# AnishDelft/ModelCompression

Hardware: AMD Instinct MI355X
Metric: images/sec (fwd+bwd, 416x416) (higher is better)
Workload: dtype fp16

## Files before the change

### include/mcamd.h

```cpp
#ifndef MCAMD_H
#define MCAMD_H

#include <stddef.h>
#include <stdint.h>

#ifdef __cplusplus
extern "C" {
#endif

#define MCAMD_OK 0
#define MCAMD_EINVAL (-1)
#define MCAMD_ELAUNCH (-2)
#define MCAMD_EWORKSPACE (-3)

int mcamd_version(void);
void mcamd_reload_config(void);
const char* mcamd_arch(void);
const char* mcamd_last_error(void);

typedef struct mcamd_conv_geom {
    int32_t B, H, W;
    int32_t ksize;
    int32_t cin;
    int32_t cout;
// ... 102 lines not shown
                       float* wq_oihw, void* stream);
int mcamd_cast_q8_train(void* src, int64_t pixels, int32_t src_ld, int32_t src_choff, int32_t C, void* dst, int32_t dst_ld,
                        int32_t dst_choff, void* stream);

int32_t mcamd_conv_fwd_q8_sparse24_ok(const mcamd_conv_geom* g);
int mcamd_q8_sparse24_elems(const mcamd_conv_geom* g, int64_t out[3]);
int mcamd_pack_q8_sparse24(const mcamd_conv_geom* g, const float* w_oihw, const float* mask_oihw, void* wq, void* idx,
                           int32_t* wexp, void* stream);
int mcamd_conv_fwd_q8_sparse24(const mcamd_conv_geom* g, const void* x8, const void* wq, const void* idx, const int32_t* wexp,
                               const mcamd_conv_epilogue* epi, int32_t y_f8, int32_t y2_f8, void* stream);

int mcamd_conv_dgrad(const mcamd_conv_geom* g, const void* dy, int32_t dy_ld, int32_t dy_choff,
                     const void* wp_dgrad, const mcamd_conv_epilogue* epi, void* stream);

typedef struct mcamd_dgrad_sums {
    float* slab;
    int32_t rows;
    int32_t ld;
    const void* act;
    int32_t act_ld, act_choff, act_pad;
    const float* scale; const float* shift; const float* mean; const float* invstd;
    float slope;
    const float* y;
    int32_t y_ld, y_choff;
    int32_t ch_lo, C;
} mcamd_dgrad_sums;
int32_t mcamd_conv_dgrad_sums_rows(const mcamd_conv_geom* g, int32_t concurrent);
int mcamd_conv_dgrad_sums(const mcamd_conv_geom* g, const void* dy, int32_t dy_ld, int32_t dy_choff,
                          const void* wp_dgrad, const mcamd_conv_epilogue* epi, const mcamd_dgrad_sums* sums, void* stream);

size_t mcamd_conv_wgrad_workspace_bytes(const mcamd_conv_geom* g);
int mcamd_conv_wgrad(const mcamd_conv_geom* g, const void* x, const void* dy, int32_t dy_ld,
                     int32_t dy_choff, const float* mask_oihw, const mcamd_chan_map* map,
                     float grad_scale, float* dw_oihw, float* dbias, void* workspace,
                     size_t workspace_bytes, void* stream);

#define MCAMD_WGRAD_GENERIC 0
#define MCAMD_WGRAD_STEM 1
#define MCAMD_WGRAD_WIN 2
#define MCAMD_WGRAD_NINE 3
#define MCAMD_WGRAD_NINE_WIDE 4
#define MCAMD_WFIN_ROW 0
#define MCAMD_WFIN_VEC 1
#define MCAMD_WFIN_GENERIC 2
#define MCAMD_WGRAD_PLAN_INFO_N 13
int mcamd_conv_wgrad_plan_info(const mcamd_conv_geom* g, int32_t has_cmap, int32_t out[MCAMD_WGRAD_PLAN_INFO_N]);
int32_t mcamd_wgrad_generic_instances(int32_t* out, int32_t cap);

int mcamd_bn_coeffs(const float* stats, int32_t stats_rows, int32_t stats_ld, int32_t C, int64_t count,
                    const float* gamma, const float* beta, float* running_mean, float* running_var,
                    float momentum, float eps, int32_t training,
                    float* scale, float* shift, float* save_mean, float* save_invstd,
                    const int32_t* chan_perm, void* stream);

int mcamd_bn_coeffs_ex(const float* stats, int32_t stats_rows, int32_t stats_ld, int32_t C, int64_t count,
                       const float* gamma, const float* beta, float* running_mean, float* running_var,
                       float momentum, float eps, int32_t training,
                       float* scale, float* shift, float* save_mean, float* save_invstd,
                       const int32_t* chan_perm, int32_t ones_channel, void* stream);

#define MCAMD_DST_PLAIN 0
#define MCAMD_DST_POOL 1
#define MCAMD_DST_REORG 2
typedef struct mcamd_act_desc {
    int32_t B, H, W, C;
    const void* y; int32_t y_ld, y_choff;
    const float* scale; const float* shift;
    float slope;
    int32_t mode;
    void* dst; int32_t dst_ld, dst_choff;
    void* dst2; int32_t dst2_ld, dst2_choff;
    int32_t y_dtype;
    int32_t planes;
    int32_t dst_plane, dst2_plane;
    int32_t dst_pad, dst2_pad;
    const float* border;
    int32_t planes2;
    void* pool_act;
    int32_t pool_act_ld, pool_act_pad;
    void* dst_q8;
    void* dst2_q8;
} mcamd_act_desc;
int mcamd_bn_act_fwd(const mcamd_act_desc* d, void* stream);

typedef struct mcamd_act_bwd_desc {
    int32_t B, H, W, C;
    const void* y; int32_t y_ld, y_choff;
    const float* scale; const float* shift; const float* mean; const float* invstd;
    float slope;
    int32_t mode;
    const void* g; int32_t g_ld, g_choff;
    const void* g2; int32_t g2_ld, g2_choff;
    void* dy; int32_t dy_ld, dy_choff;
    float* dgamma; float* dbeta;
    float grad_scale;
    const float* dy_keep;
    const int32_t* chan_perm;
    int32_t y_dtype;
    int32_t* overflow;
    int32_t dy_pad;
    int32_t skip_dead_param_grads;
    const void* act;
    int32_t act_ld, act_choff, act_pad;
    const void* pool_out;
    int32_t pool_out_ld, pool_out_choff, pool_out_pad;
    const float* sums;
    int32_t sums_rows, sums_ld;
} mcamd_act_bwd_desc;
size_t mcamd_bn_act_bwd_workspace_bytes(const mcamd_act_bwd_desc* d);
int mcamd_bn_act_bwd(const mcamd_act_bwd_desc* d, void* workspace, size_t workspace_bytes, void* stream);

typedef struct mcamd_fold_desc {
    const float* w; const float* mask;
    const int32_t* rows; const int32_t* cols;
    const float* beta; float slope;
    int32_t n, cin_t, cin_k, cin_aug, ksize;
} mcamd_fold_desc;
int mcamd_fold_weights(const mcamd_fold_desc* d, float* waug, void* stream);
typedef struct mcamd_fold_job {
    mcamd_fold_desc d;
    float* waug;
    int64_t first_block;
} mcamd_fold_job;
int mcamd_fold_weights_many(const mcamd_fold_job* jobs_dev, int32_t njobs, int64_t total_blocks, void* stream);
int mcamd_unfold_wgrad(const mcamd_fold_desc* d, const float* dwaug, float* dw_oihw, float* prod_dbeta,
                       float* prod_dgamma, int32_t accumulate, void* stream);

typedef struct mcamd_stem_block_desc {
    int32_t B, H, W;
    const void* x;
    const void* wp;
    const float* gamma; const float* beta;
    float* running_mean; float* running_var;
    float momentum, eps;
    int32_t training;
    float* scale; float* shift; float* save_mean; float* save_invstd;
    float slope;
    void* dst; int32_t dst_ld, dst_choff;
    const void* g; int32_t g_ld, g_choff;
    const float* mask;
    float grad_scale;
    float* dw;
    float* dgamma; float* dbeta;
    int32_t cout;
    int32_t planes;
    const void* x_lo;
    const void* wp_lo;
} mcamd_stem_block_desc;
size_t mcamd_stem_block_workspace_bytes(void);
int mcamd_stem_block_fwd(const mcamd_stem_block_desc* d, void* workspace, size_t workspace_bytes, void* stream);
int mcamd_stem_block_bwd(const mcamd_stem_block_desc* d, void* workspace, size_t workspace_bytes, void* stream);
int32_t mcamd_stem_block_stats_rows(const mcamd_stem_block_desc* d);
int mcamd_stem_block_stats(const mcamd_stem_block_desc* d, float* stats, int32_t stats_rows, int32_t stats_ld, void* stream);

int mcamd_nchw_f32_to_padded_nhwc_f16(const float* src, int32_t B, int32_t C, int32_t H, int32_t W,
                                      float mul, void* dst, int32_t dst_ld, int32_t dst_choff, int32_t* overflow,
                                      void* stream);
int mcamd_nchw_f32_to_padded_nhwc_f16_pad(const float* src, int32_t B, int32_t C, int32_t H, int32_t W,
                                          float mul, void* dst, int32_t dst_ld, int32_t dst_choff, int32_t pad,
                                          int32_t* overflow, void* stream);
int mcamd_nchw_f32_to_padded_nhwc_f16_split(const float* src, int32_t B, int32_t C, int32_t H, int32_t W,
                                            void* dst, int32_t dst_ld, int32_t dst_choff, int32_t plane, void* stream);

int mcamd_nchw_f32_to_nhwc4_split(const float* src, int32_t B, int32_t H, int32_t W, void* hi, void* lo, void* stream);
int mcamd_pack_stem_split(const float* w_oihw, const float* mask_oihw, int32_t cout, void* wp_hi, void* wp_lo, void* stream);

// ... 104 lines not shown
```

### modelcompression_amd/_lib.py

```python
import ctypes as C
import os

_HERE = os.path.dirname(os.path.abspath(__file__))
LIB_PATH = os.path.join(_HERE, "libmcamd.so")


class McamdError(RuntimeError):
    pass


class ConvGeom(C.Structure):
    _fields_ = [("B", C.c_int32), ("H", C.c_int32), ("W", C.c_int32), ("ksize", C.c_int32),
                ("cin", C.c_int32), ("cout", C.c_int32), ("x_ld", C.c_int32), ("x_choff", C.c_int32),
                ("stem", C.c_int32), ("pad", C.c_int32), ("x_wrap", C.c_int32), ("x_f8", C.c_int32), ("x_f8_wexp", C.c_int32)]


class ConvEpilogue(C.Structure):
    _fields_ = [("mode", C.c_int32), ("y_ld", C.c_int32), ("y_choff", C.c_int32),
                ("y", C.c_void_p), ("bias", C.c_void_p), ("stats", C.c_void_p),
                ("stats_rows", C.c_int32), ("stats_ld", C.c_int32),
                ("scale", C.c_void_p), ("shift", C.c_void_p), ("slope", C.c_float), ("overflow", C.c_void_p),
                ("dst_mode", C.c_int32), ("y2", C.c_void_p), ("y2_ld", C.c_int32), ("y2_choff", C.c_int32),
                ("concurrent", C.c_int32)]

# ... 92 lines not shown
                ("gt_box", C.c_void_p), ("gt_cls", C.c_void_p), ("gt_difficult", C.c_void_p), ("gt_count", C.c_void_p),
                ("image_size", C.c_void_p),
                ("keys", C.c_void_p), ("flags", C.c_void_p), ("capacity", C.c_int64), ("counters", C.c_void_p)]


class FoldJob(C.Structure):
    _fields_ = [("d", FoldDesc), ("waug", C.c_void_p), ("first_block", C.c_int64)]


class AugmentDesc(C.Structure):
    _fields_ = [("src_off", C.c_int64), ("tmp_off", C.c_int64),
                ("src_w", C.c_int32), ("src_h", C.c_int32), ("crop_x", C.c_int32), ("crop_y", C.c_int32),
                ("crop_w", C.c_int32), ("crop_h", C.c_int32), ("flip", C.c_int32),
                ("hk", C.c_int32), ("vk", C.c_int32), ("hcoef_off", C.c_int32), ("vcoef_off", C.c_int32),
                ("lut_off", C.c_int32)]


class AugmentBatch(C.Structure):
    _fields_ = [("desc", C.c_void_p), ("desc_dev", C.c_void_p),
                ("src", C.c_void_p), ("src_bytes", C.c_int64),
                ("coef", C.c_void_p), ("coef_elems", C.c_int64),
                ("lut", C.c_void_p), ("lut_bytes", C.c_int64),
                ("tmp", C.c_void_p), ("tmp_bytes", C.c_int64),
                ("out", C.c_void_p), ("B", C.c_int32), ("H", C.c_int32), ("W", C.c_int32)]


EPI_RAW_F16, EPI_NCHW_F32, EPI_PAD_F16, EPI_RAW_F32 = 0, 1, 2, 3
DST_PLAIN, DST_POOL, DST_REORG = 0, 1, 2
WGRAD_GENERIC, WGRAD_STEM, WGRAD_WIN, WGRAD_NINE, WGRAD_NINE_WIDE = 0, 1, 2, 3, 4
WFIN_ROW, WFIN_VEC, WFIN_GENERIC = 0, 1, 2
WGRAD_PLAN_INFO_N = 13

_P, _I32, _I64, _F, _SZ = C.c_void_p, C.c_int32, C.c_int64, C.c_float, C.c_size_t
SIGNATURES = {
    "mcamd_version": (C.c_int, []),
    "mcamd_arch": (C.c_char_p, []),
    "mcamd_last_error": (C.c_char_p, []),
    "mcamd_reload_config": (None, []),
    "mcamd_conv_stats_rows": (_I32, [C.POINTER(ConvGeom)]),
    "mcamd_conv_stats_rows_mode": (_I32, [C.POINTER(ConvGeom), _I32]),
    "mcamd_conv_fwd_f8_ok": (_I32, [C.POINTER(ConvGeom)]),
    "mcamd_conv_tile_info": (C.c_int, [C.POINTER(ConvGeom), _I32, C.POINTER(_I32)]),
    "mcamd_conv_route_info": (C.c_int, [C.POINTER(ConvGeom), _I32, _I32, _I32, _I32, C.POINTER(_I32)]),
    "mcamd_packed_elems_fwd": (_I64, [C.POINTER(ConvGeom)]),
    "mcamd_packed_elems_dgrad": (_I64, [C.POINTER(ConvGeom)]),
    "mcamd_pack_weights": (C.c_int, [C.POINTER(ConvGeom), _P, _P, C.POINTER(ChanMap), _P, _P, _P]),
    "mcamd_pack_weights_many": (C.c_int, [_P, _I32, _I64, _P]),
    "mcamd_conv_fwd": (C.c_int, [C.POINTER(ConvGeom), _P, _P, C.POINTER(ConvEpilogue), _P]),
    "mcamd_conv_fwd_sparse24_ok": (_I32, [C.POINTER(ConvGeom)]),
    "mcamd_sparse24_elems": (C.c_int, [C.POINTER(ConvGeom), C.POINTER(_I64)]),
    "mcamd_pack_sparse24": (C.c_int, [C.POINTER(ConvGeom), _P, _P, _P, _P, _P]),
    "mcamd_conv_fwd_sparse24": (C.c_int, [C.POINTER(ConvGeom), _P, _P, _P, C.POINTER(ConvEpilogue), _P]),
    "mcamd_conv_fwd_splitk_info": (C.c_int, [C.POINTER(ConvGeom), _I32, _I32, _I32, C.POINTER(SplitkInfo)]),
    "mcamd_conv_fwd_splitk": (C.c_int, [C.POINTER(ConvGeom), _P, _P, C.POINTER(ConvEpilogue), _I32, _P, _SZ, _P]),
    "mcamd_conv_fwd_q8_ok": (_I32, [C.POINTER(ConvGeom)]),
    "mcamd_q8_elems": (C.c_int, [C.POINTER(ConvGeom), C.POINTER(_I64)]),
    "mcamd_pack_q8": (C.c_int, [C.POINTER(ConvGeom), _P, _P, _P, _P, _P]),
    "mcamd_conv_fwd_q8": (C.c_int, [C.POINTER(ConvGeom), _P, _P, _P, C.POINTER(ConvEpilogue), _I32, _I32, _P]),
    "mcamd_conv_fwd_q8_slim_ok": (_I32, [C.POINTER(ConvGeom)]),
    "mcamd_q8_slim_elems": (C.c_int, [C.POINTER(ConvGeom), C.POINTER(_I64)]),
    "mcamd_pack_q8_slim": (C.c_int, [C.POINTER(ConvGeom), _P, _P, _P, _P, _P]),
    "mcamd_conv_fwd_q8_slim": (C.c_int, [C.POINTER(ConvGeom), _P, _P, _P, C.POINTER(ConvEpilogue), _P, _I32, _I32, _I32, _P]),
    "mcamd_conv_fwd_q8_sparse24_ok": (_I32, [C.POINTER(ConvGeom)]),
    "mcamd_q8_sparse24_elems": (C.c_int, [C.POINTER(ConvGeom), C.POINTER(_I64)]),
    "mcamd_pack_q8_sparse24": (C.c_int, [C.POINTER(ConvGeom), _P, _P, _P, _P, _P, _P]),
    "mcamd_conv_fwd_q8_sparse24": (C.c_int, [C.POINTER(ConvGeom), _P, _P, _P, _P, C.POINTER(ConvEpilogue), _I32, _I32, _P]),
    "mcamd_cast_q8": (C.c_int, [_P, _I64, _I32, _I32, _I32, _P, _I32, _I32, _P]),
    "mcamd_conv_fwd_q8_stats_rows": (_I32, [C.POINTER(ConvGeom)]),
    "mcamd_fakequant_q8": (C.c_int, [C.POINTER(ConvGeom), _P, _P, _P, _P, _P]),
    "mcamd_cast_q8_train": (C.c_int, [_P, _I64, _I32, _I32, _I32, _P, _I32, _I32, _P]),
    "mcamd_conv_dgrad": (C.c_int, [C.POINTER(ConvGeom), _P, _I32, _I32, _P, C.POINTER(ConvEpilogue), _P]),
    "mcamd_conv_dgrad_sums_rows": (_I32, [C.POINTER(ConvGeom), _I32]),
    "mcamd_conv_dgrad_sums": (C.c_int, [C.POINTER(ConvGeom), _P, _I32, _I32, _P, C.POINTER(ConvEpilogue), C.POINTER(DgradSums), _P]),
    "mcamd_conv_wgrad_workspace_bytes": (_SZ, [C.POINTER(ConvGeom)]),
    "mcamd_conv_wgrad": (C.c_int, [C.POINTER(ConvGeom), _P, _P, _I32, _I32, _P, C.POINTER(ChanMap), _F, _P, _P, _P, _SZ, _P]),
    "mcamd_conv_wgrad_plan_info": (C.c_int, [C.POINTER(ConvGeom), _I32, C.POINTER(_I32)]),
    "mcamd_wgrad_generic_instances": (_I32, [C.POINTER(_I32), _I32]),
    "mcamd_bn_coeffs": (C.c_int, [_P, _I32, _I32, _I32, _I64, _P, _P, _P, _P, _F, _F, _I32, _P, _P, _P, _P, _P, _P]),
    "mcamd_bn_coeffs_ex": (C.c_int, [_P, _I32, _I32, _I32, _I64, _P, _P, _P, _P, _F, _F, _I32, _P, _P, _P, _P, _P, _I32, _P]),
    "mcamd_fold_weights": (C.c_int, [C.POINTER(FoldDesc), _P, _P]),
    "mcamd_fold_weights_many": (C.c_int, [_P, _I32, _I64, _P]),
    "mcamd_unfold_wgrad": (C.c_int, [C.POINTER(FoldDesc), _P, _P, _P, _P, _I32, _P]),
    "mcamd_bn_act_fwd": (C.c_int, [C.POINTER(ActDesc), _P]),
    "mcamd_bn_act_bwd_workspace_bytes": (_SZ, [C.POINTER(ActBwdDesc)]),
    "mcamd_bn_act_bwd": (C.c_int, [C.POINTER(ActBwdDesc), _P, _SZ, _P]),
    "mcamd_stem_block_workspace_bytes": (_SZ, []),
    "mcamd_stem_block_fwd": (C.c_int, [C.POINTER(StemBlockDesc), _P, _SZ, _P]),
    "mcamd_stem_block_bwd": (C.c_int, [C.POINTER(StemBlockDesc), _P, _SZ, _P]),
    "mcamd_stem_block_stats_rows": (_I32, [C.POINTER(StemBlockDesc)]),
    "mcamd_stem_block_stats": (C.c_int, [C.POINTER(StemBlockDesc), _P, _I32, _I32, _P]),
    "mcamd_nchw_f32_to_nhwc4_split": (C.c_int, [_P, _I32, _I32, _I32, _P, _P, _P]),
    "mcamd_pack_stem_split": (C.c_int, [_P, _P, _I32, _P, _P, _P]),
    "mcamd_nchw_f32_to_padded_nhwc_f16": (C.c_int, [_P, _I32, _I32, _I32, _I32, _F, _P, _I32, _I32, _P, _P]),
    "mcamd_nchw_f32_to_padded_nhwc_f16_pad": (C.c_int, [_P, _I32, _I32, _I32, _I32, _F, _P, _I32, _I32, _I32, _P, _P]),
    "mcamd_nchw_f32_to_padded_nhwc_f16_split": (C.c_int, [_P, _I32, _I32, _I32, _I32, _P, _I32, _I32, _I32, _P]),
    "mcamd_stem_conv_f32_stats_rows": (_I32, []),
    "mcamd_stem_conv_f32": (C.c_int, [_P, _I32, _I32, _I32, _P, _P, _I32, _P, _P, _I32, _P, _I32, _I32, _P]),
    "mcamd_region_loss_workspace_bytes": (_SZ, [_I32]),
    "mcamd_region_loss": (C.c_int, [C.POINTER(RegionDesc), _P, _P, _P, _P, _SZ, _P]),
    "mcamd_region_decode": (C.c_int, [C.POINTER(DetectDesc), _P, _P, _P]),
    "mcamd_nms": (C.c_int, [_P, _P, _I32, _I32, _F, _P, _P, _P]),
    "mcamd_detect": (C.c_int, [C.POINTER(DetectDesc), _P, _P, _P, _P, _P, _P]),
    "mcamd_voc_match": (C.c_int, [C.POINTER(VocMatchDesc), _P]),
    "mcamd_voc_ap": (C.c_int, [_P, _P, _P, _I64, _P, _I32, _P, _P, _P, _P]),
    "mcamd_augment": (C.c_int, [C.POINTER(AugmentBatch), _P]),
    "mcamd_augment_tables": (C.c_int, [_P, _P, _P, _I32, _I32, _I32, _P, _I64, _P, _I64, _P]),
    "mcamd_plan_begin": (C.c_int, [C.POINTER(_P), _I32]),
    "mcamd_plan_mark": (_I32, []),
    "mcamd_plan_end": (_P, []),
    "mcamd_plan_segments": (_I32, [_P]),
    "mcamd_plan_launches": (_I32, [_P]),
    "mcamd_plan_run": (C.c_int, [_P, _I32, _I32, C.POINTER(_P), _I32]),
    "mcamd_plan_destroy": (None, [_P]),
    "mcamd_stream_wait": (C.c_int, [_P, _P]),
    "mcamd_memset_zero": (C.c_int, [_P, _SZ, _P]),
    "mcamd_step_flags": (C.c_int, [_P, _I32, _P, _P, _P, _P, _P]),
    "mcamd_kth_magnitude_workspace_bytes": (_SZ, []),
    "mcamd_kth_magnitude": (C.c_int, [C.POINTER(_P), C.POINTER(_I64), _I32, _I64, _P, _P, _SZ, _P]),
    "mcamd_magnitude_mask": (C.c_int, [_P, _I64, _P, _P, _P]),
    "mcamd_filter_scores_workspace_bytes": (_SZ, [_I32]),
    "mcamd_filter_scores": (C.c_int, [_P, _I32, _I32, _I32, _I32, _P, _P, _SZ, _P]),
    "mcamd_filter_mean_square": (C.c_int, [_P, _I32, _I32, _I32, _I32, _P, _P, _SZ, _P]),
    "mcamd_filter_mask": (C.c_int, [_P, _I32, _I64, _P, _P]),
    "mcamd_count_zeros": (C.c_int, [_P, _I64, _P, _P]),
    "mcamd_masked_residual": (C.c_int, [_P, _P, _I64, _P, _P]),
    "mcamd_nm_mask": (C.c_int, [_P, _P, _I32, _I32, _I32, _I32, _I32, _P, _P]),
    "mcamd_nm_violations": (C.c_int, [_P, _I32, _I32, _I32, _P, _P]),
}

_lib = None


def lib():
    global _lib
    if _lib is None:
        if not os.path.exists(LIB_PATH):
            raise McamdError(
                "libmcamd.so is missing (%s). Build it with `python -m modelcompression_amd.build`; "
                "modelcompression_amd has no CPU/PyTorch fallback for its compute path." % LIB_PATH)
        import torch
        h = C.CDLL(LIB_PATH)
        for name, (res, args) in SIGNATURES.items():
            fn = getattr(h, name)
            fn.restype = res
            fn.argtypes = args
        _lib = h
    return _lib


def reload_config():
    lib().mcamd_reload_config()


def check(rc, what=""):
    if rc != 0:
        msg = lib().mcamd_last_error().decode()
        raise McamdError("%s failed (%d): %s" % (what or "mcamd call", rc, msg))


def ptr(t):
    return None if t is None else C.c_void_p(t.data_ptr())


def stream_ptr():
    import torch
    return C.c_void_p(torch.cuda.current_stream().cuda_stream)
# ... 1 lines not shown
```

### modelcompression_amd/build.py

```python
import os
import subprocess
import sys
from concurrent.futures import ThreadPoolExecutor

HERE = os.path.dirname(os.path.abspath(__file__))
CSRC = os.path.join(HERE, "csrc")
OUT = os.path.join(HERE, "libmcamd.so")
HIPCC = os.environ.get("HIPCC", "/opt/rocm/bin/hipcc")
ARCH = "gfx950"
COMMON = ["--offload-arch=" + ARCH, "-O3", "-fPIC", "-std=c++17", "-Wall", "-Wno-unused-variable",
          "-fhip-fp32-correctly-rounded-divide-sqrt"]
SOURCES = {
    "api.hip": [],
    "conv_igemm.hip": [],
    "conv_igemm_pp.hip": [],
    "conv_sparse.hip": [],
    "conv_splitk.hip": [],
    "conv_q8.hip": [],
    "conv_q8_sparse.hip": [],
    "conv_stem.hip": [],
    "conv_stem_block.hip": [],
    "conv_stem_f32.hip": [],
    "conv_small.hip": [],
    "conv_win.hip": [],
    "conv_wres.hip": [],
    "conv_wgrad.hip": [],
    "conv_wgrad_stem.hip": [],
    "bn_act.hip": [],
    "fold.hip": [],
    "plan.hip": [],
    "region_loss.hip": [],
    "prune.hip": ["-ffp-contract=off"],
    "augment.hip": ["-ffp-contract=off"],
    "detect.hip": ["-ffp-contract=off"],
    "voc_eval.hip": ["-ffp-contract=off"],
}


def _stale(target, deps):
    if not os.path.exists(target):
        return True
    t = os.path.getmtime(target)
    return any(os.path.getmtime(d) > t for d in deps)


def build(force=False, verbose=False):
    headers = [os.path.join(CSRC, f) for f in os.listdir(CSRC) if f.endswith(".h")]
    headers.append(os.path.join(os.path.dirname(HERE), "include", "mcamd.h"))
    objdir = os.path.join(CSRC, "build")
    os.makedirs(objdir, exist_ok=True)
    jobs = []
    for src, extra in SOURCES.items():
        s = os.path.join(CSRC, src)
        o = os.path.join(objdir, src.replace(".hip", ".o"))
        if force or _stale(o, [s] + headers):
            jobs.append([HIPCC] + COMMON + extra + ["-c", s, "-o", o])

    def run(cmd):
        if verbose:
            print(" ".join(cmd))
        r = subprocess.run(cmd, capture_output=True, text=True)
        if r.returncode != 0:
            raise RuntimeError("hipcc failed:\n%s\n%s" % (" ".join(cmd), r.stderr))
        return r.stderr

    with ThreadPoolExecutor(max_workers=4) as ex:
        for err in ex.map(run, jobs):
            if verbose and err.strip():
                print(err)
    objs = [os.path.join(objdir, s.replace(".hip", ".o")) for s in SOURCES]
    if force or jobs or _stale(OUT, objs):
        run([HIPCC, "--offload-arch=" + ARCH, "-shared", "-fPIC", "-o", OUT] + objs)
    return OUT


if __name__ == "__main__":
    print(build(force="--force" in sys.argv, verbose=True))
```

### modelcompression_amd/csrc/api.hip

```cpp
#include <stdarg.h>
#include <stdlib.h>
#include <string.h>

#include "kernels.h"

static thread_local char g_err[512] = "";

void mcamd_set_error(const char* fmt, ...) {
    va_list ap;
    va_start(ap, fmt);
    vsnprintf(g_err, sizeof(g_err), fmt, ap);
    va_end(ap);
}

int g_mcamd_env_generation = 0;
int McamdEnvSlot::get(const char* name, int dflt) {
    const int g = __atomic_load_n(&g_mcamd_env_generation, __ATOMIC_ACQUIRE);
    if (gen != g) {
        const char* s = getenv(name);
        has = s && *s ? 1 : 0;
        val = has ? atoi(s) : 0;
        __atomic_store_n(&gen, g, __ATOMIC_RELEASE);
    }
    return has ? val : dflt;
}
extern "C" void mcamd_reload_config(void) { __atomic_add_fetch(&g_mcamd_env_generation, 1, __ATOMIC_ACQ_REL); }

extern "C" int mcamd_version(void) { return 101; }
extern "C" const char* mcamd_arch(void) { return "gfx950"; }
extern "C" const char* mcamd_last_error(void) { return g_err; }

static int cin_tap_of(const mcamd_conv_geom* g) { return g->stem ? 32 : round_up_int(g->cin, 32); }
static int ntaps_of(const mcamd_conv_geom* g) { return g->stem ? 3 : g->ksize * g->ksize; }
static int cout_p_of(const mcamd_conv_geom* g) { return round_up_int(g->cout, 32); }
static int pw_of(const mcamd_conv_geom* g) { return g->pad ? 1 : 2; }
static long long padded_pixels(const mcamd_conv_geom* g) {
    const int pw = pw_of(g);
    return (long long)g->B * (g->H + pw) * (g->W + pw) + (pw == 1 ? g->W + 2 : 0);
}

static int check_geom(const mcamd_conv_geom* g, const char* what) {
    MCAMD_REQUIRE(g, "%s: null geometry", what);
    MCAMD_REQUIRE(g->B > 0 && g->H > 0 && g->W > 0 && g->cin > 0 && g->cout > 0, "%s: non-positive dimension", what);
    MCAMD_REQUIRE(g->ksize == 1 || g->ksize == 3, "%s: ksize %d unsupported (1 or 3)", what, g->ksize);
    MCAMD_REQUIRE((long long)g->B * g->H * g->W < (1ll << 31), "%s: more than 2^31 output pixels", what);
    MCAMD_REQUIRE(g->pad == 0 || (g->pad == 1 && !g->stem), "%s: pad must be 0 or 1 (and 0 for the stem layer)", what);
    if (g->stem) {
        MCAMD_REQUIRE(g->cin == 3 && g->ksize == 3 && g->x_ld == 4 && g->x_choff == 0,
                      "%s: stem form needs cin=3, ksize=3, x_ld=4, x_choff=0", what);
    } else {
        MCAMD_REQUIRE(g->x_ld % 8 == 0 && g->x_choff % 8 == 0, "%s: x_ld / x_choff must be multiples of 8", what);
        const int span = g->x_wrap > 0 ? g->x_wrap : cin_tap_of(g);
        MCAMD_REQUIRE(g->x_choff + span <= g->x_ld, "%s: x channel slice [%d, %d) exceeds x_ld %d", what,
                      g->x_choff, g->x_choff + span, g->x_ld);
    }
    if (g->x_f8 != 0) {
        MCAMD_REQUIRE(!g->stem && g->x_wrap == 0 && g->x_f8 > 0 && g->x_f8 % 64 == 0 && g->cin == 2 * g->x_f8 && g->x_choff == 0,
                      "%s: x_f8 %d needs cin = 2 P with P %% 64 == 0, no x_wrap, x_choff 0 (cin %d, x_choff %d)", what, g->x_f8, g->cin,
                      g->x_choff);
        MCAMD_REQUIRE(g->x_f8_wexp >= -24 && g->x_f8_wexp <= 40, "%s: x_f8_wexp %d outside [-24, 40]", what, g->x_f8_wexp);
    }
    if (g->x_wrap != 0) {
        const int ct = cin_tap_of(g), kb = ct % 64 == 0 ? 64 : 32;
        MCAMD_REQUIRE(!g->stem && g->x_wrap > 0 && g->x_wrap % 64 == 0 && g->x_wrap % kb == 0 && g->cin == g->x_wrap / 2 * 3 && ct == g->cin,
                      "%s: x_wrap %d needs cin = 3 P, x_wrap = 2 P, P %% 32 == 0 (cin %d)", what, g->x_wrap, g->cin);
    }
    return MCAMD_OK;
}

static void fill_taps(int ksize, int stem, int row_stride, int ld, int* taps) {
    if (stem) {
        for (int ty = 0; ty < 3; ++ty) taps[ty] = ty * row_stride;
    } else if (ksize == 3) {
        for (int ty = 0; ty < 3; ++ty)
            for (int tx = 0; tx < 3; ++tx) taps[ty * 3 + tx] = ty * row_stride + tx * ld;
    } else {
        taps[0] = row_stride + ld;
    }
}

extern "C" int64_t mcamd_packed_elems_fwd(const mcamd_conv_geom* g) {
    if (!g) return 0;
    return (int64_t)round_up_int(g->cout, 256) * ntaps_of(g) * cin_tap_of(g);
}
extern "C" int64_t mcamd_packed_elems_dgrad(const mcamd_conv_geom* g) {
// ... 374 lines not shown
    if (mcamd_win3x3_ok(mode, stats, M, n, ct, ktot, g->H, g->W))
        return {ROUTE_WIN3X3, 32, round_up_int(n, 16), 64, 0};
    if (fwd && g->x_f8 > 0 && mode == MCAMD_EPI_RAW_F32) ct = ct / 2 * 3, ktot = ktot / 2 * 3;
    return mcamd_igemm_route(M, n, ct, ktot, mode == MCAMD_EPI_RAW_F16, dir == DIR_DGRAD_CONCURRENT);
}

static int launch_route(IgemmArgs& a, const ConvRoute& r, const mcamd_conv_geom* g, hipStream_t st) {
    switch (r.kernel) {
    case ROUTE_STEM: {
        StemArgs q;
        q.x = a.x, q.w = a.w, q.y = (half_t*)a.y, q.stats = a.stats;
        q.y_ld = a.y_ld, q.y_choff = a.y_choff, q.stats_ld = a.stats_ld;
        q.H = g->H, q.W = g->W, q.HW = a.HW, q.M = a.M;
        return mcamd_stem_launch(q, g->cout, r.rows, st);
    }
    case ROUTE_WRES: return mcamd_wres_launch(a, g->B, r.rows, st);
    case ROUTE_SMALL3X3_SPLIT: return mcamd_small3x3_split_launch(a, r.rows, st);
    case ROUTE_SMALL3X3: return mcamd_small3x3_launch(a, r.rows, st);
    case ROUTE_WIN3X3: return mcamd_win3x3_launch(a, st);
    default: return mcamd_igemm_launch(a, r, st);
    }
}

extern "C" int32_t mcamd_conv_stats_rows_mode(const mcamd_conv_geom* g, int32_t mode) {
    if (!g) return 0;
    return conv_route(g, DIR_FWD, mode == MCAMD_EPI_RAW_F32 ? MCAMD_EPI_RAW_F32 : MCAMD_EPI_RAW_F16, MCAMD_DST_PLAIN, true).rows;
}

extern "C" int32_t mcamd_conv_stats_rows(const mcamd_conv_geom* g) { return mcamd_conv_stats_rows_mode(g, MCAMD_EPI_RAW_F16); }

extern "C" int32_t mcamd_conv_fwd_f8_ok(const mcamd_conv_geom* g) {
    if (!g || g->x_f8 <= 0 || g->x_f8 % 64 != 0 || g->cin != 2 * g->x_f8 || g->stem || g->x_wrap != 0 || g->x_choff != 0) return 0;
    return conv_route(g, DIR_FWD, MCAMD_EPI_RAW_F32, MCAMD_DST_PLAIN, true).kernel == ROUTE_PP ? 1 : 0;
}

extern "C" int mcamd_conv_tile_info(const mcamd_conv_geom* g, int32_t dgrad, int32_t out[4]) {
    if (check_geom(g, "conv_tile_info")) return MCAMD_EINVAL;
    MCAMD_REQUIRE(out, "conv_tile_info: null output");
    const bool f32 = !dgrad && (g->x_wrap > 0 || g->x_f8 > 0);
    const ConvRoute r = conv_route(g, dgrad, f32 ? MCAMD_EPI_RAW_F32 : MCAMD_EPI_RAW_F16, MCAMD_DST_PLAIN, !dgrad);
    out[0] = r.bm, out[1] = r.bn, out[2] = r.bk, out[3] = r.kernel;
    return MCAMD_OK;
}

extern "C" int mcamd_conv_route_info(const mcamd_conv_geom* g, int32_t dir, int32_t mode, int32_t dst_mode, int32_t stats,
                                     int32_t out[5]) {
    if (check_geom(g, "conv_route_info")) return MCAMD_EINVAL;
    MCAMD_REQUIRE(out, "conv_route_info: null output");
    MCAMD_REQUIRE(dir == DIR_FWD || dir == DIR_DGRAD || dir == DIR_DGRAD_CONCURRENT, "conv_route_info: bad direction %d", dir);
    MCAMD_REQUIRE(mode >= MCAMD_EPI_RAW_F16 && mode <= MCAMD_EPI_RAW_F32, "conv_route_info: bad epilogue mode %d", mode);
    MCAMD_REQUIRE(dst_mode == MCAMD_DST_PLAIN || dst_mode == MCAMD_DST_POOL || dst_mode == MCAMD_DST_REORG,
                  "conv_route_info: bad dst_mode %d", dst_mode);
    const ConvRoute r = conv_route(g, dir, mode, dst_mode, stats != 0);
    out[0] = r.bm, out[1] = r.bn, out[2] = r.bk, out[3] = r.kernel, out[4] = r.rows;
    return MCAMD_OK;
}

extern "C" int mcamd_conv_fwd(const mcamd_conv_geom* g, const void* x, const void* wp_fwd, const mcamd_conv_epilogue* epi,
                              void* stream) {
    if (mcamd_recording()) {
        MCAMD_REQUIRE(g && epi, "conv_fwd: null geometry / epilogue");
        const mcamd_conv_geom g_ = *g;
        const mcamd_conv_epilogue e_ = *epi;
        return mcamd_rec_push(stream, [=](void* s) { return mcamd_conv_fwd(&g_, x, wp_fwd, &e_, s); });
    }
    if (check_geom(g, "conv_fwd")) return MCAMD_EINVAL;
    MCAMD_REQUIRE(x && wp_fwd && epi, "conv_fwd: null input / epilogue");
    IgemmArgs a;
    fill_operand(a, g, x, wp_fwd, g->x_ld, g->x_choff, g->cout, cin_tap_of(g), g->stem);
    MCAMD_REQUIRE(g->x_wrap == 0 || epi->mode == MCAMD_EPI_RAW_F32 || epi->mode == MCAMD_EPI_NCHW_F32,
                  "conv_fwd: x_wrap goes with the fp32 epilogues (modes 3 and 1)");
    if (g->x_wrap > 0) a.wrap = g->x_wrap;
    if (g->x_f8 > 0) a.f8_from = (g->x_f8 / a.kb) * a.ntaps * (a.kb / 32);
    a.f8_sb = (127 - (MCAMD_F8_SXL + g->x_f8_wexp)) * 0x01010101;
    const ConvRoute r = conv_route(g, DIR_FWD, epi->mode, epi->dst_mode, epi->stats != nullptr);
    if (g->x_f8 > 0) {
        MCAMD_REQUIRE(epi->mode == MCAMD_EPI_RAW_F32, "conv_fwd: x_f8 goes with the fp32 epilogue (mode 3)");
        MCAMD_REQUIRE(r.kernel == ROUTE_PP, "conv_fwd: no fp8-correction kernel for this shape (mcamd_conv_fwd_f8_ok)");
    }
    if (fill_epilogue(a, epi, g->cout, "conv_fwd", r.rows)) return MCAMD_EINVAL;
    return launch_route(a, r, g, (hipStream_t)stream);
}

extern "C" int32_t mcamd_conv_fwd_sparse24_ok(const mcamd_conv_geom* g) {
    if (!g || g->stem || g->x_wrap != 0 || g->x_f8 != 0 || (g->ksize != 1 && g->ksize != 3)) return 0;
    if (g->B <= 0 || g->H <= 0 || g->W <= 0 || g->cin <= 0 || g->cout <= 0) return 0;
    if (g->cin % 4 != 0 || g->cout % 8 != 0 || (long long)g->B * g->H * g->W >= (1ll << 31)) return 0;
    if (g->pad != 0 && g->pad != 1) return 0;
    if (g->x_ld % 8 != 0 || g->x_choff % 8 != 0 || g->x_choff + cin_tap_of(g) > g->x_ld) return 0;
    return 1;
}

extern "C" int mcamd_sparse24_elems(const mcamd_conv_geom* g, int64_t out[2]) {
    MCAMD_REQUIRE(g && out, "sparse24_elems: null argument");
    MCAMD_REQUIRE(mcamd_conv_fwd_sparse24_ok(g), "sparse24_elems: geometry has no 2:4 form (mcamd_conv_fwd_sparse24_ok)");
    const long long npad = round_up_int(g->cout, 256), ktot = (long long)ntaps_of(g) * cin_tap_of(g);
    out[0] = npad * ktot / 2;
    out[1] = npad * ktot / 16;
    return MCAMD_OK;
}

extern "C" int mcamd_pack_sparse24(const mcamd_conv_geom* g, const float* w_oihw, const float* mask_oihw, void* wsp, void* idx,
                                   void* stream) {
    if (mcamd_recording()) {
        MCAMD_REQUIRE(g, "pack_sparse24: null geometry");
        const mcamd_conv_geom g_ = *g;
        return mcamd_rec_push(stream, [=](void* s) { return mcamd_pack_sparse24(&g_, w_oihw, mask_oihw, wsp, idx, s); });
    }
    MCAMD_REQUIRE(g && mcamd_conv_fwd_sparse24_ok(g), "pack_sparse24: geometry has no 2:4 form (mcamd_conv_fwd_sparse24_ok)");
    MCAMD_REQUIRE(w_oihw && wsp && idx, "pack_sparse24: null pointer");
    const int ct = cin_tap_of(g);
    return mcamd_pack_sparse24_launch(w_oihw, mask_oihw, wsp, idx, g->cout, g->cin, ntaps_of(g), ct, kblock_of(ct),
                                      (hipStream_t)stream);
}

extern "C" int mcamd_conv_fwd_sparse24(const mcamd_conv_geom* g, const void* x, const void* wsp, const void* idx,
                                       const mcamd_conv_epilogue* epi, void* stream) {
    if (mcamd_recording()) {
        MCAMD_REQUIRE(g && epi, "conv_fwd_sparse24: null geometry / epilogue");
        const mcamd_conv_geom g_ = *g;
        const mcamd_conv_epilogue e_ = *epi;
        return mcamd_rec_push(stream, [=](void* s) { return mcamd_conv_fwd_sparse24(&g_, x, wsp, idx, &e_, s); });
    }
    if (check_geom(g, "conv_fwd_sparse24")) return MCAMD_EINVAL;
    MCAMD_REQUIRE(mcamd_conv_fwd_sparse24_ok(g), "conv_fwd_sparse24: geometry has no 2:4 form (mcamd_conv_fwd_sparse24_ok)");
    MCAMD_REQUIRE(x && wsp && idx, "conv_fwd_sparse24: null input");
    MCAMD_REQUIRE(epi && epi->mode == MCAMD_EPI_PAD_F16, "conv_fwd_sparse24: epilogue mode 2 (MCAMD_EPI_PAD_F16) only");
    IgemmArgs a;
    fill_operand(a, g, x, wsp, g->x_ld, g->x_choff, g->cout, cin_tap_of(g), 0);
    if (fill_epilogue(a, epi, g->cout, "conv_fwd_sparse24", 0)) return MCAMD_EINVAL;
    return mcamd_sparse24_launch(a, idx, (hipStream_t)stream);
}

static int splitk_plan_for(const mcamd_conv_geom* g, int mode, int dst_mode, int slices, const char* what, SplitkPlan* p) {
    MCAMD_REQUIRE(g, "%s: null geometry", what);
    MCAMD_REQUIRE(g->stem == 0, "%s: stem %d: the first layer has no split-K form", what, g->stem);
    MCAMD_REQUIRE(g->pad == 0, "%s: pad %d: the shared-halo form is not accepted (pad must be 0)", what, g->pad);
    MCAMD_REQUIRE(g->x_wrap == 0, "%s: x_wrap %d: split operands have no split-K form", what, g->x_wrap);
    MCAMD_REQUIRE(g->x_f8 == 0, "%s: x_f8 %d: the fp8 correction form has no split-K form", what, g->x_f8);
    if (check_geom(g, what)) return MCAMD_EINVAL;
    MCAMD_REQUIRE(mode == MCAMD_EPI_PAD_F16 || mode == MCAMD_EPI_RAW_F16,
                  "%s: epilogue mode %d: modes 2 (MCAMD_EPI_PAD_F16) and 0 (MCAMD_EPI_RAW_F16) only", what, mode);
    MCAMD_REQUIRE(dst_mode == MCAMD_DST_PLAIN || (mode == MCAMD_EPI_PAD_F16 && (dst_mode == MCAMD_DST_POOL || dst_mode == MCAMD_DST_REORG)),
                  "%s: bad dst_mode %d for epilogue mode %d", what, dst_mode, mode);
    MCAMD_REQUIRE(slices >= 0, "%s: slices %d is negative", what, slices);
    const int ct = cin_tap_of(g);
    *p = mcamd_splitk_plan((long long)g->B * g->H * g->W, g->cout, ct, ntaps_of(g) * ct, slices);
    MCAMD_REQUIRE(p->slices >= 1 && p->slices <= p->chunks, "%s: slices %d outside [1, chunks = %d]", what, p->slices, p->chunks);
    return MCAMD_OK;
}

extern "C" int mcamd_conv_fwd_splitk_info(const mcamd_conv_geom* g, int32_t mode, int32_t dst_mode, int32_t slices,
                                          mcamd_splitk_info* out) {
    MCAMD_REQUIRE(out, "conv_fwd_splitk_info: null output");
    SplitkPlan p;
    if (splitk_plan_for(g, mode, dst_mode, slices, "conv_fwd_splitk_info", &p)) return MCAMD_EINVAL;
    out->slices = p.slices;
    out->bm = p.bm, out->bn = p.bn, out->bk = p.bk;
    out->chunks = p.chunks;
    out->tiles = p.tiles;
    out->workspace_bytes = (int64_t)p.slices * p.slab_elems * (int64_t)sizeof(float);
    return MCAMD_OK;
}

extern "C" int mcamd_conv_fwd_splitk(const mcamd_conv_geom* g, const void* x, const void* wp_fwd, const mcamd_conv_epilogue* epi,
                                     int32_t slices, void* workspace, size_t workspace_bytes, void* stream) {
// ... 379 lines not shown
```

### modelcompression_amd/csrc/bn_act.hip

```cpp
#include "common.h"
#include "conv_epi.h"

constexpr int RED_CPB = 8, RED_RG = 128;

__device__ __forceinline__ double shfl_xor_f64(double v, int m) {
    int lo = __double2loint(v), hi = __double2hiint(v);
    lo = __shfl_xor(lo, m);
    hi = __shfl_xor(hi, m);
    return __hiloint2double(hi, lo);
}

__device__ __forceinline__ void block_reduce2(double& a, double& b, double (*red)[16][RED_CPB]) {
    const int lane = threadIdx.x & 63, wave = threadIdx.x >> 6, cx = threadIdx.x & (RED_CPB - 1);
#pragma unroll
    for (int m = RED_CPB; m < 64; m <<= 1) {
        a += shfl_xor_f64(a, m);
        b += shfl_xor_f64(b, m);
    }
    if (lane < RED_CPB) {
        red[0][wave][cx] = a;
        red[1][wave][cx] = b;
    }
    __syncthreads();
    if (threadIdx.x < RED_CPB) {
        a = b = 0.0;
        for (int w = 0; w < 16; ++w) {
            a += red[0][w][cx];
            b += red[1][w][cx];
        }
    }
}

__global__ __launch_bounds__(1024) void bn_coeffs_kernel(const float* stats, int rows, int ld, int C, double count,
                                                         const float* gamma, const float* beta, float* rmean,
                                                         float* rvar, float momentum, float eps, int training,
                                                         float* scale, float* shift, float* save_mean,
                                                         float* save_invstd, const int* perm, int ones_channel) {
    __shared__ double red[2][16][RED_CPB];
    const int cx = threadIdx.x & (RED_CPB - 1), ry = threadIdx.x / RED_CPB;
    const int c = blockIdx.x * RED_CPB + cx;
    double s1 = 0.0, s2 = 0.0;
    if (training && c < C) {
        for (int p = ry; p < rows; p += RED_RG) {
            s1 += (double)stats[((long long)p * 2 + 0) * ld + c];
            s2 += (double)stats[((long long)p * 2 + 1) * ld + c];
        }
    }
    block_reduce2(s1, s2, red);
    if (ry != 0 || c >= C) return;
    const int pc = perm ? perm[c] : c;
    double mean, var;
    if (training) {
        mean = s1 / count;
        var = s2 / count - mean * mean;
        if (var < 0.0) var = 0.0;
        double unbiased = count > 1.0 ? var * count / (count - 1.0) : var;
        rmean[pc] = (float)((1.0 - momentum) * (double)rmean[pc] + (double)momentum * mean);
        rvar[pc] = (float)((1.0 - momentum) * (double)rvar[pc] + (double)momentum * unbiased);
    } else {
        mean = rmean[pc];
        var = rvar[pc];
    }
    double invstd = 1.0 / sqrt(var + (double)eps);
    float sc = (float)((double)gamma[pc] * invstd);
    scale[c] = sc;
    shift[c] = (float)((double)beta[pc] - mean * (double)sc);
    if (c == ones_channel) scale[c] = 0.f, shift[c] = 1.f;
    if (save_mean) save_mean[c] = (float)mean;
    if (save_invstd) save_invstd[c] = (float)invstd;
}

struct ActArgs {
    const void* y;
    const float* scale;
    const float* shift;
    half_t* dst;
    half_t* dst2;
    int B, H, W, C;
    int y_ld, y_choff, dst_ld, dst_choff, dst2_ld, dst2_choff;
    float slope;
    long long items;
    const float* border;
    int dst_plane, dst2_plane;
    int dst_pw, dst2_pw;
    int dst2_pl;
    half_t* pool_act;
    int pool_act_ld, pool_act_pw;
    char* dst_q8;
    char* dst2_q8;
};

__device__ __forceinline__ void load8(const half_t* p, float* v) {
    h8_t h = *(const h8_t*)p;
#pragma unroll
    for (int i = 0; i < 8; ++i) v[i] = (float)h[i];
}
__device__ __forceinline__ half_t sat_half(float v) {
    return (half_t)fminf(fmaxf(v, -65504.f), 65504.f);
}
__device__ __forceinline__ void store8(half_t* p, const float* v) {
    h8_t h;
#pragma unroll
    for (int i = 0; i < 8; ++i) h[i] = sat_half(v[i]);
    *(h8_t*)p = h;
}
__device__ __forceinline__ void loadf8(const float* p, float* v) {
    f32x4_t a = *(const f32x4_t*)p, b = *(const f32x4_t*)(p + 4);
#pragma unroll
    for (int i = 0; i < 4; ++i) {
        v[i] = a[i];
        v[4 + i] = b[i];
    }
}
template <bool Y32>
__device__ __forceinline__ void load_y(const void* y, long long idx, float* v) {
    if (Y32) loadf8((const float*)y + idx, v);
    else load8((const half_t*)y + idx, v);
}
template <int PL>
__device__ __forceinline__ void store_act(half_t* p, int plane, const float* v, int ci = 0) {
    h8_t hi;
#pragma unroll
    for (int i = 0; i < 8; ++i) hi[i] = sat_half(v[i]);
    *(h8_t*)p = hi;
    if (PL == 4) {
        float ql[8], q8[8];
#pragma unroll
        for (int i = 0; i < 8; ++i) {
            ql[i] = fminf(fmaxf((v[i] - (float)hi[i]) * (float)(1 << MCAMD_F8_SXL), -448.f), 448.f);
            q8[i] = fminf(fmaxf(v[i] * (float)(1 << MCAMD_F8_SX8), -448.f), 448.f);
        }
        int wl[2], w8[2];
#pragma unroll
        for (int i = 0; i < 2; ++i) {
            wl[i] = __builtin_amdgcn_cvt_pk_fp8_f32(ql[4 * i], ql[4 * i + 1], 0, false);
            wl[i] = __builtin_amdgcn_cvt_pk_fp8_f32(ql[4 * i + 2], ql[4 * i + 3], wl[i], true);
            w8[i] = __builtin_amdgcn_cvt_pk_fp8_f32(q8[4 * i], q8[4 * i + 1], 0, false);
            w8[i] = __builtin_amdgcn_cvt_pk_fp8_f32(q8[4 * i + 2], q8[4 * i + 3], w8[i], true);
        }
        char* b = (char*)(p - ci + plane) + ci;
        typedef int i32x2_t __attribute__((ext_vector_type(2)));
        *(i32x2_t*)b = i32x2_t{wl[0], wl[1]};
        *(i32x2_t*)(b + plane) = i32x2_t{w8[0], w8[1]};
    } else if (PL >= 2) {
        h8_t lo;
#pragma unroll
        for (int i = 0; i < 8; ++i) lo[i] = (half_t)(v[i] - (float)hi[i]);
        *(h8_t*)(p + plane) = lo;
        if (PL == 3) *(h8_t*)(p + 2 * plane) = hi;
    }
}
__device__ __forceinline__ void store_act_q8(half_t* p, char* q, long long off, const float* v) {
    if (!q) {
        store_act<1>(p + off, 0, v);
        return;
    }
    i32x2_t o;
    o[0] = e4m3_bytes4(v), o[1] = e4m3_bytes4(v + 4);
    *(i32x2_t*)(q + off) = o;
    h8_t h = q8_to_f16(o[0], o[1]);
#pragma unroll
    for (int i = 0; i < 8; ++i) h[i] = h[i] * (half_t)0.5f;
    *(h8_t*)(p + off) = h;
}
__device__ __forceinline__ unsigned short half_prev_bits(unsigned short b) {
    if (b == 0x0000 || b == 0x8000) return 0x8001;
    return (b & 0x8000) ? (unsigned short)(b + 1) : (unsigned short)(b - 1);
}
template <int PL>
__device__ __forceinline__ void store_act2(int pl2, half_t* p, int plane, const float* v, int ci) {
    if (PL < 2 || pl2 == PL) store_act<PL>(p, plane, v, ci);
    else if (pl2 == 4) store_act<4>(p, plane, v, ci);
    else if (pl2 == 3) store_act<3>(p, plane, v, ci);
    else if (pl2 == 2) store_act<2>(p, plane, v, ci);
    else store_act<1>(p, plane, v, ci);
}

__device__ __forceinline__ int border_class(int h, int w, int H, int W) {
    return (h == 0 ? 1 : 0) | (h == H - 1 ? 2 : 0) | (w == 0 ? 4 : 0) | (w == W - 1 ? 8 : 0);
}

template <int MODE, bool FIXED, bool Y32, int PL, bool Q8 = false>
__global__ __launch_bounds__(256) void bn_act_fwd_kernel(ActArgs a) {
    const int CH = a.C >> 3;
    int c8 = (threadIdx.x % CH) * 8;
    float sc[8], sh[8];
    if (FIXED) {
        loadf8(a.scale + c8, sc);
        loadf8(a.shift + c8, sh);
    }
    const int Ho = a.H >> 1, Wo = a.W >> 1;
    for (long long item = (long long)blockIdx.x * 256 + threadIdx.x; item < a.items; item += (long long)gridDim.x * 256) {
        long long pix = item / CH;
        if (!FIXED) {
            c8 = (int)(item - pix * CH) * 8;
            loadf8(a.scale + c8, sc);
            loadf8(a.shift + c8, sh);
        }
        if (MODE == MCAMD_DST_PLAIN) {
            int b = (int)(pix / (a.H * a.W));
            int rem = (int)(pix - (long long)b * a.H * a.W);
            int h = rem / a.W, w = rem - h * a.W;
            float v[8];
            load_y<Y32>(a.y, pix * a.y_ld + a.y_choff + c8, v);
            if (a.border) {
                float bb[8];
                loadf8(a.border + border_class(h, w, a.H, a.W) * a.C + c8, bb);
#pragma unroll
                for (int i = 0; i < 8; ++i) v[i] += bb[i];
            }
#pragma unroll
            for (int i = 0; i < 8; ++i) {
                float z = v[i] * sc[i] + sh[i];
                v[i] = z > 0.f ? z : z * a.slope;
            }
            if (Q8) store_act_q8(a.dst, a.dst_q8, pad_off(b, h, w, a.H, a.W, a.dst_ld, a.dst_pw) + a.dst_choff + c8, v);
            else store_act<PL>(a.dst + pad_off(b, h, w, a.H, a.W, a.dst_ld, a.dst_pw) + a.dst_choff + c8, a.dst_plane, v, a.dst_choff + c8);
        } else {
            int b = (int)(pix / (Ho * Wo));
            int rem = (int)(pix - (long long)b * Ho * Wo);
            int ho = rem / Wo, wo = rem - ho * Wo;
            float act[4][8];
#pragma unroll
            for (int k = 0; k < 4; ++k) {
                int h = 2 * ho + (k >> 1), w = 2 * wo + (k & 1);
                long long sp = ((long long)b * a.H + h) * a.W + w;
                load_y<Y32>(a.y, sp * a.y_ld + a.y_choff + c8, act[k]);
                if (a.border) {
                    float bb[8];
                    loadf8(a.border + border_class(h, w, a.H, a.W) * a.C + c8, bb);
#pragma unroll
                    for (int i = 0; i < 8; ++i) act[k][i] += bb[i];
                }
#pragma unroll
                for (int i = 0; i < 8; ++i) {
                    float z = act[k][i] * sc[i] + sh[i];
                    act[k][i] = z > 0.f ? z : z * a.slope;
                }
                if (Q8) {
                    if (a.dst2) store_act_q8(a.dst2, a.dst2_q8, pad_off(b, h, w, a.H, a.W, a.dst2_ld, a.dst2_pw) + a.dst2_choff + c8, act[k]);
                } else if (a.dst2) store_act2<PL>(a.dst2_pl, a.dst2 + pad_off(b, h, w, a.H, a.W, a.dst2_ld, a.dst2_pw) + a.dst2_choff + c8, a.dst2_plane, act[k], a.dst2_choff + c8);
            }
            long long dp = pad_off(b, ho, wo, Ho, Wo, a.dst_ld, a.dst_pw) + a.dst_choff;
            if (MODE == MCAMD_DST_POOL) {
                float m[8];
#pragma unroll
                for (int i = 0; i < 8; ++i) m[i] = fmaxf(fmaxf(act[0][i], act[1][i]), fmaxf(act[2][i], act[3][i]));
                if (Q8) store_act_q8(a.dst, a.dst_q8, dp + c8, m);
                else store_act<PL>(a.dst + dp + c8, a.dst_plane, m, a.dst_choff + c8);
                if (!Q8 && a.pool_act) {
                    typedef unsigned short us8_t __attribute__((ext_vector_type(8)));
                    us8_t hb[4];
#pragma unroll
                    for (int i = 0; i < 8; ++i) {
                        int arg = 0;
                        float best = act[0][i];
#pragma unroll
                        for (int k = 1; k < 4; ++k) {
                            const bool gt = act[k][i] > best;
                            best = gt ? act[k][i] : best, arg = gt ? k : arg;
                        }
                        const unsigned short top = __builtin_bit_cast(unsigned short, sat_half(best));
                        const unsigned short below = half_prev_bits(top);
#pragma unroll
                        for (int k = 0; k < 4; ++k) {
                            const unsigned short hk = __builtin_bit_cast(unsigned short, sat_half(act[k][i]));
                            hb[k][i] = (k != arg && hk == top) ? below : hk;
                        }
                    }
                    half_t* q0 = a.pool_act + pad_off(b, 2 * ho, 2 * wo, a.H, a.W, a.pool_act_ld, a.pool_act_pw) + c8;
                    const long long qrow = (long long)(a.W + a.pool_act_pw) * a.pool_act_ld;
                    *(us8_t*)q0 = hb[0];
                    *(us8_t*)(q0 + a.pool_act_ld) = hb[1];
                    *(us8_t*)(q0 + qrow) = hb[2];
                    *(us8_t*)(q0 + qrow + a.pool_act_ld) = hb[3];
                }
            } else {
#pragma unroll
                for (int k = 0; k < 4; ++k) {
                    if (Q8) store_act_q8(a.dst, a.dst_q8, dp + k * a.C + c8, act[k]);
                    else store_act<PL>(a.dst + dp + k * a.C + c8, a.dst_plane, act[k], a.dst_choff + k * a.C + c8);
                }
            }
        }
    }
}

struct ActBwdArgs {
    const void* y;
    const float* scale;
    const float* shift;
    const float* mean;
    const float* invstd;
    const half_t* g;
    const half_t* g2;
    half_t* dy;
    float* slab;
    const float* coef;
    const float* dy_keep;
    int* overflow;
    int B, H, W, C;
    int y_ld, y_choff, g_ld, g_choff, g2_ld, g2_choff, dy_ld, dy_choff;
    float slope;
    long long items;
    int dy_pw;
    const half_t* act;
    int act_ld, act_choff, act_pw;
    const half_t* pool_out;
    int pool_out_ld, pool_out_choff, pool_out_pw;
};

__device__ __forceinline__ void block_partials_to_slab(const float (&sb)[8], const float (&sg)[8], int CH, float* slab, int C) {
    constexpr int PITCH = 264;
    __shared__ float red[16 * PITCH];
#pragma unroll
    for (int i = 0; i < 8; ++i) {
        red[i * PITCH + threadIdx.x] = sb[i];
        red[(8 + i) * PITCH + threadIdx.x] = sg[i];
    }
    __syncthreads();
    const int reps = 256 / CH;
// ... 1102 lines not shown
```

### modelcompression_amd/csrc/conv_epi.h

```cpp
#pragma once
#include "kernels.h"

__device__ __forceinline__ void split_image(int p, int HW, int& b, int& hw) {
    b = p / HW;
    hw = p - b * HW;
}
__device__ __forceinline__ void split_pixel(int p, int HW, int W, int& b, int& h, int& w) {
    int r;
    split_image(p, HW, b, r);
    h = r / W;
    w = r - h * W;
}

__device__ __forceinline__ void tile_pixel(const IgemmArgs& __restrict__ a, bool pooled, int m, int& b, int& h, int& w) {
    if (pooled) {
        const int Wo = a.W >> 1, q = m & 3;
        int ho, wo;
        split_pixel(m >> 2, (a.H >> 1) * Wo, Wo, b, ho, wo);
        h = 2 * ho + (q >> 1);
        w = 2 * wo + (q & 1);
    } else {
        split_pixel(m, a.HW, a.W, b, h, w);
    }
}
// ... 47 lines not shown
template <int ROWS, int COLS, int PITCH, int NT>
__device__ __forceinline__ void store_pad_tile(const IgemmArgs& __restrict__ a, const char* bt, const half_t* ht, bool y_f8, bool y2_f8,
                                               int mt, int nt, int tid) {
    constexpr int CH = COLS / 8;
    if (a.dst_mode == MCAMD_DST_PLAIN) {
        for (int slot = tid; slot < ROWS * CH; slot += NT) {
            const int row = slot / CH, ch = slot - row * CH;
            const int m = mt * ROWS + row;
            const int n0 = nt * COLS + ch * 8;
            if (m < a.M && n0 < a.N) {
                int b, h, w;
                split_pixel(m, a.HW, a.W, b, h, w);
                put8(a.y, y_f8, pad_off(b, h, w, a.H, a.W, a.y_ld) + a.y_choff + n0, bt, ht, row * PITCH + ch * 8);
            }
        }
        return;
    }
    const int Wo = a.W >> 1, Ho = a.H >> 1, HWo = Ho * Wo;
    if (a.dst_mode == MCAMD_DST_POOL) {
        const bool has2 = a.y2 != nullptr;
        for (int slot = tid; slot < (ROWS / 4) * CH; slot += NT) {
            const int pr = slot / CH, ch = slot - pr * CH;
            const int idx = mt * (ROWS / 4) + pr;
            const int n0 = nt * COLS + ch * 8;
            if (4 * idx < a.M && n0 < a.N) {
                int b, ho, wo;
                split_pixel(idx, HWo, Wo, b, ho, wo);
                const long long off = pad_off(b, ho, wo, Ho, Wo, a.y_ld) + a.y_choff + n0;
                if (y_f8) {
                    unsigned k0 = 0, k1 = 0;
#pragma unroll
                    for (int q = 0; q < 4; ++q) {
                        const i32x2_t v = *(const i32x2_t*)(bt + (4 * pr + q) * PITCH + ch * 8);
                        k0 = e4m3_max4(k0, e4m3_key((unsigned)v[0]));
                        k1 = e4m3_max4(k1, e4m3_key((unsigned)v[1]));
                    }
                    i32x2_t mx;
                    mx[0] = (int)e4m3_unkey(k0), mx[1] = (int)e4m3_unkey(k1);
                    *(i32x2_t*)((char*)a.y + off) = mx;
                } else {
                    h8_t v[4];
#pragma unroll
                    for (int q = 0; q < 4; ++q) v[q] = *(const h8_t*)(ht + (4 * pr + q) * PITCH + ch * 8);
                    h8_t mx;
#pragma unroll
                    for (int e = 0; e < 8; ++e) {
                        const half_t m01 = v[0][e] > v[1][e] ? v[0][e] : v[1][e], m23 = v[2][e] > v[3][e] ? v[2][e] : v[3][e];
                        mx[e] = m01 > m23 ? m01 : m23;
                    }
                    *(h8_t*)((half_t*)a.y + off) = mx;
                }
                if (has2) {
#pragma unroll
                    for (int q = 0; q < 4; ++q)
                        put8(a.y2, y2_f8, pad_off(b, 2 * ho + (q >> 1), 2 * wo + (q & 1), a.H, a.W, a.y2_ld) + a.y2_choff + n0,
                             bt, ht, (4 * pr + q) * PITCH + ch * 8);
                }
            }
        }
    } else {
        for (int slot = tid; slot < ROWS * CH; slot += NT) {
            const int row = slot / CH, ch = slot - row * CH;
            const int m = mt * ROWS + row;
            const int n0 = nt * COLS + ch * 8;
            if (m < a.M && n0 < a.N) {
                int b, ho, wo;
                split_pixel(m >> 2, HWo, Wo, b, ho, wo);
                put8(a.y, y_f8, pad_off(b, ho, wo, Ho, Wo, a.y_ld) + a.y_choff + (m & 3) * a.N + n0, bt, ht, row * PITCH + ch * 8);
            }
        }
    }
}

template <int ROWS, int COLS, int NT>
__device__ __forceinline__ void store_raw_tile(const IgemmArgs& __restrict__ a, const half_t* ct, int mt, int nt, int tid) {
    constexpr int CH = COLS / 8;
    half_t* y = (half_t*)a.y;
    for (int slot = tid; slot < ROWS * CH; slot += NT) {
        const int row = slot / CH, ch = slot - row * CH;
        const int m = mt * ROWS + row;
        const int n0 = nt * COLS + ch * 8;
        if (m < a.M && n0 < a.N) *(h8_t*)(y + (long long)m * a.y_ld + a.y_choff + n0) = *(const h8_t*)(ct + row * COLS + ch * 8);
    }
}

template <class T>
__device__ __forceinline__ const T* pin_here(const T* p) {
    asm volatile("" : "+s"(p));
    return p;
}
__host__ __device__ constexpr int sums_vals(int cols, int nt) { return (2 * cols + nt - 1) / nt; }
__host__ __device__ constexpr size_t sums_lds_bytes(int nt) { return (size_t)16 * (nt + 8) * sizeof(float); }

__host__ __device__ constexpr int sums_slots(int rows, int cols, int nt) { return rows * (cols / 8) / nt; }
__host__ __device__ constexpr int sums_early(int rows, int cols, int nt) {
    return rows * cols >= 256 * 256 && sums_slots(rows, cols, nt) > 8 ? 8 : sums_slots(rows, cols, nt);
}

template <int ROWS, int COLS, int NT>
__device__ __forceinline__ void sums_prefetch(const IgemmArgs& __restrict__ a, int mt, int nt, int tid,
                                              h8_t (&aq)[sums_early(ROWS, COLS, NT)]) {
    constexpr int CH = COLS / 8, RSTEP = NT / CH, NSLOT = sums_early(ROWS, COLS, NT);
    static_assert(NT % CH == 0 && (ROWS * CH) % NT == 0, "a thread keeps its 8 channels for all its slots");
    const int ch = tid % CH, row0 = tid / CH;
    const int n0 = nt * COLS + ch * 8;
    const int c = n0 - a.bsum.ch_lo;
    const bool live = n0 < a.N && c >= 0 && c < a.bsum.C;
    const half_t* act = pin_here(a.bsum.act) + a.bsum.act_choff + c;
    int m = mt * ROWS + row0;
    int b, h, w;
    split_pixel(m, a.HW, a.W, b, h, w);
    const int sb_ = RSTEP / a.HW, srem = RSTEP - sb_ * a.HW;
    const int sh_ = srem / a.W, sw_ = srem - sh_ * a.W;
#pragma unroll
    for (int k = 0; k < NSLOT; ++k) {
#pragma unroll
        for (int i = 0; i < 8; ++i) aq[k][i] = (half_t)0.f;
        if (live && m < a.M) aq[k] = *(const h8_t*)(act + pad_off(b, h, w, a.H, a.W, a.bsum.act_ld, a.bsum.act_pw));
        m += RSTEP;
        w += sw_;
        if (w >= a.W) w -= a.W, ++h;
        h += sh_;
        if (h >= a.H) h -= a.H, ++b;
        b += sb_;
    }
}

template <int ROWS, int COLS, int NT>
__device__ __forceinline__ void store_raw_tile_sums(const IgemmArgs& __restrict__ a, char* smem, int mt, int nt, int tid,
                                                    const h8_t (&aq)[sums_early(ROWS, COLS, NT)],
                                                    float (&tot)[sums_vals(COLS, NT)]) {
    constexpr int CH = COLS / 8, RSTEP = NT / CH, NSLOT = sums_slots(ROWS, COLS, NT), PITCH = NT + 8;
    constexpr int EARLY = sums_early(ROWS, COLS, NT);
    const half_t* ct = (const half_t*)smem;
    half_t* y = (half_t*)a.y;
    const int ch = tid % CH, row0 = tid / CH;
    const int n0 = nt * COLS + ch * 8;
    const int c = n0 - a.bsum.ch_lo;
    const bool col_ok = n0 < a.N;
    const bool live = col_ok && c >= 0 && c < a.bsum.C;
    float sb[8], sg[8], off[8], mul[8];
    bool usey[8];
    bool need_y = false;
#pragma unroll
    for (int i = 0; i < 8; ++i) sb[i] = sg[i] = 0.f, off[i] = 0.f, mul[i] = 0.f, usey[i] = false;
    if (live) {
        const float *scp = pin_here(a.bsum.scale) + c, *shp = pin_here(a.bsum.shift) + c;
        const float *mup = pin_here(a.bsum.mean) + c, *isp = pin_here(a.bsum.invstd) + c;
        float sc[8], sh[8], mu[8], is[8];
#pragma unroll
        for (int i = 0; i < 8; ++i) sc[i] = scp[i], sh[i] = shp[i], mu[i] = mup[i], is[i] = isp[i];
        need_y = act_xhat_source(sc, sh, mu, is, a.bsum.y != nullptr, off, mul, usey);
    }
    const float slope = a.bsum.slope, inv_slope = 1.0f / slope;
#pragma unroll
    for (int k = 0; k < NSLOT; ++k) {
        const int row = row0 + k * RSTEP, m = mt * ROWS + row;
        if (!col_ok || m >= a.M) continue;
        const h8_t gq = *(const h8_t*)(ct + row * COLS + ch * 8);
        *(h8_t*)(y + (long long)m * a.y_ld + a.y_choff + n0) = gq;
        if (!live) continue;
        h8_t av8;
        if (k < EARLY) {
            av8 = aq[k];
        } else {
            int b, h, w;
// ... 136 lines not shown
```

### modelcompression_amd/csrc/conv_igemm.hip

```cpp
#include "kernels.h"
#include "conv_epi.h"
#include <stdlib.h>


template <int BM, int BN, int WM, int WN, int BK, int NSTAGE, int EPI>
__global__ __launch_bounds__((BM / WM) * (BN / WN) * 64,
                              (BN >= 128 ? (NSTAGE * BK <= 96 ? 3 : 2) : (BN >= 64 ? 3 : 4)))
void igemm_kernel(IgemmArgs a) {
    constexpr int WAVES_N = BN / WN;
    constexpr int NT = (BM / WM) * (BN / WN) * 64;
    constexpr int CPR = BK / 8;
    constexpr int A_SLOTS = BM * CPR, B_SLOTS = BN * CPR;
    constexpr int A_IT = (A_SLOTS + NT - 1) / NT, B_IT = (B_SLOTS + NT - 1) / NT;
    constexpr int TM = WM / 32, TN = WN / 32;
    constexpr int STAGE_BYTES = (A_SLOTS + B_SLOTS) * 16;
    constexpr int DMIN = A_SLOTS / NT + B_SLOTS / NT;
    static_assert(A_SLOTS % 64 == 0 && B_SLOTS % 64 == 0, "whole waves per DMA instruction");
    static_assert(NSTAGE >= 2 && NSTAGE <= 4 && DMIN * (NSTAGE - 2) < 64, "vmcnt immediate range");

    extern __shared__ __attribute__((aligned(16))) char smem[];

    const int tid = threadIdx.x;
    const int lane = tid & 63;
    const int wave = __builtin_amdgcn_readfirstlane(tid >> 6);
// ... 67 lines not shown
                int wslot = it * NT + wave * 64;
                if (wslot < B_SLOTS) glds16(a.w + bbase[it] + (long long)q * BK, sb + wslot * 16);
            }
        };

        __syncthreads();
#pragma unroll
        for (int p = 0; p < NSTAGE - 1; ++p)
            if (p < nchunks) stage(p, p);
        int sidx = 0;
        for (int q = 0; q < nchunks; ++q) {
            int issued = q + NSTAGE - 1;
            if (issued > nchunks) issued = nchunks;
            const int inflight = issued - q - 1;
            if (NSTAGE == 2 || inflight == 0) wait_vmcnt<0>();
            else if (inflight == 1) wait_vmcnt<DMIN>();
            else wait_vmcnt<(NSTAGE > 3 ? 2 * DMIN : DMIN)>();
            __builtin_amdgcn_s_barrier();
            if (q + NSTAGE - 1 < nchunks) {
                int ns = sidx + NSTAGE - 1;
                if (ns >= NSTAGE) ns -= NSTAGE;
                stage(q + NSTAGE - 1, ns);
            }
            const char* sa = smem + sidx * STAGE_BYTES;
            const char* sb = sa + A_SLOTS * 16;
            sidx = sidx + 1 == NSTAGE ? 0 : sidx + 1;
            constexpr int KS = BK / 16;
            constexpr int NSET = (TM * TN <= 4) ? 2 : 1;
            h8_t af[NSET][TM], bf[NSET][TN];
            auto load_frags = [&](int s, int set) {
                const int chunk = 2 * s + (lane >> 5);
#pragma unroll
                for (int i = 0; i < TM; ++i) {
                    int row = wm * WM + i * 32 + (lane & 31);
                    af[set][i] = *(const h8_t*)(sa + (row * CPR + (chunk ^ swz<CPR>(row))) * 16);
                }
#pragma unroll
                for (int j = 0; j < TN; ++j) {
                    int row = wn * WN + j * 32 + (lane & 31);
                    bf[set][j] = *(const h8_t*)(sb + (row * CPR + (chunk ^ swz<CPR>(row))) * 16);
                }
            };
            if (NSET == 2) load_frags(0, 0);
#pragma unroll
            for (int s = 0; s < KS; ++s) {
                if (NSET == 2) {
                    if (s + 1 < KS) load_frags(s + 1, (s + 1) & 1);
                    __builtin_amdgcn_sched_barrier(0);
                } else {
                    load_frags(s, 0);
                }
                constexpr int M1 = NSET - 1;
#pragma unroll
                for (int i = 0; i < TM; ++i)
#pragma unroll
                    for (int j = 0; j < TN; ++j)
                        acc[i][j] = __builtin_amdgcn_mfma_f32_32x32x16_f16(af[s & M1][i], bf[s & M1][j], acc[i][j], 0, 0, 0);
                if (NSET == 2) __builtin_amdgcn_sched_barrier(0);
            }
        }

        if constexpr (EPI == MCAMD_EPI_NCHW_F32) {
            float* y = (float*)a.y;
#pragma unroll
            for (int i = 0; i < TM; ++i)
#pragma unroll
                for (int r = 0; r < 16; ++r) {
                    int m = mt * BM + wm * WM + i * 32 + mfma32_row(r, lane);
                    if (m < a.M) {
                        int b, hw;
                        split_image(m, a.HW, b, hw);
#pragma unroll
                        for (int j = 0; j < TN; ++j) {
                            int n = nt * BN + wn * WN + j * 32 + (lane & 31);
                            if (n < a.N) {
                                float v = acc[i][j][r];
                                if (a.bias) v += a.bias[n];
                                y[((long long)b * a.N + n) * a.HW + hw] = v;
                            }
                        }
                    }
                }
        } else if constexpr (EPI == MCAMD_EPI_RAW_F32) {
            float* y = (float*)a.y;
            const int mlim = a.M - mt * BM;
#pragma unroll
            for (int j = 0; j < TN; ++j) {
                const int n = nt * BN + wn * WN + j * 32 + (lane & 31);
#pragma unroll
                for (int i = 0; i < TM; ++i)
#pragma unroll
                    for (int r = 0; r < 16; ++r) {
                        const int row = wm * WM + i * 32 + mfma32_row(r, lane);
                        const float v = acc[i][j][r];
                        if (row < mlim) {
                            if (n < a.N) y[(long long)(mt * BM + row) * a.y_ld + a.y_choff + n] = v;
                            s1[j] += v;
                            s2[j] += v * v;
                        }
                    }
            }
        } else {
            h8_t aq[SUMS ? sums_early(BM, BN, NT) : 1];
            if constexpr (SUMS) sums_prefetch<BM, BN, NT>(a, mt, nt, tid, aq);
            __syncthreads();
            half_t* ct = (half_t*)smem;
            const int mlim = a.M - mt * BM;
#pragma unroll
            for (int j = 0; j < TN; ++j) {
                const int col = wn * WN + j * 32 + (lane & 31);
                float sc = 1.f, sh = 0.f;
                if constexpr (EPI == MCAMD_EPI_PAD_F16) {
                    int n = nt * BN + col;
                    if (n < a.N) {
                        if (a.scale) sc = a.scale[n];
                        if (a.shift) sh = a.shift[n];
                    }
                }
#pragma unroll
                for (int i = 0; i < TM; ++i)
#pragma unroll
                    for (int r = 0; r < 16; ++r) {
                        const int row = wm * WM + i * 32 + mfma32_row(r, lane);
                        float v = acc[i][j][r];
                        if constexpr (EPI == MCAMD_EPI_PAD_F16) {
                            v = v * sc + sh;
                            v = v > 0.f ? v : v * a.slope;
                        }
                        half_t hv = (half_t)fminf(fmaxf(v, -65504.f), 65504.f);
                        sat |= fabsf(v) > 65504.f;
                        ct[row * BN + col] = hv;
                        if (EPI == MCAMD_EPI_RAW_F16 && a.stats) {
                            float fv = (row < mlim) ? (float)hv : 0.f;
                            s1[j] += fv;
                            s2[j] += fv * fv;
                        }
                    }
            }
            __syncthreads();
            if constexpr (EPI == MCAMD_EPI_PAD_F16) store_pad_tile<BM, BN, BN, NT>(a, nullptr, ct, false, false, mt, nt, tid);
            else if constexpr (SUMS) store_raw_tile_sums<BM, BN, NT>(a, smem, mt, nt, tid, aq, tot);
            else store_raw_tile<BM, BN, NT>(a, ct, mt, nt, tid);
        }
    }

    if (sat && a.overflow) atomicOr(a.overflow, 1);
    if constexpr (SUMS) store_tile_sums_slab<BN, NT>(a, pslot, nt, tid, tot);
    if ((EPI == MCAMD_EPI_RAW_F16 || EPI == MCAMD_EPI_RAW_F32) && a.stats) {
#pragma unroll
        for (int j = 0; j < TN; ++j) {
            s1[j] += __shfl_xor(s1[j], 32);
            s2[j] += __shfl_xor(s2[j], 32);
        }
        __syncthreads();
        float* red = (float*)smem;
        if (lane < 32) {
#pragma unroll
            for (int j = 0; j < TN; ++j) {
                red[(wm * 2 + 0) * BN + wn * WN + j * 32 + lane] = s1[j];
                red[(wm * 2 + 1) * BN + wn * WN + j * 32 + lane] = s2[j];
            }
        }
        __syncthreads();
        for (int t = tid; t < 2 * BN; t += NT) {
            int which = t / BN, col = t - which * BN;
            float v = 0.f;
#pragma unroll
            for (int k = 0; k < BM / WM; ++k) v += red[(k * 2 + which) * BN + col];
            a.stats[((long long)pslot * 2 + which) * a.stats_ld + nt * BN + col] = v;
        }
    }
}

struct TileCfg {
    int bm, bn, bk;
    int kind;
};

static TileCfg pick_tile(long long M, int n, int cin_tap, int ktot, bool raw_epilogue = true, bool concurrent = false) {
    TileCfg t;
    t.kind = 0;
    if (raw_epilogue && mcamd_small3x3_ok(M, n, cin_tap, ktot)) {
        t.bm = 32, t.bn = round_up_int(n, 32), t.bk = cin_tap, t.kind = 4;
        return t;
    }
    {
        const int pp = MCAMD_ENV_INT("MCAMD_PP", 1);
        if (pp && ktot >= 256 && n >= 128 && M >= 256) {
            bool use = pp == 2;
            int bm = 256, bn = 256;
            if (pp == 1 && ktot >= 1152) {
                double best_cost = -1.0, best_span = 0.0;
                const int bms[2] = {256, 192}, bns[2] = {256, 128};
                for (int cn = 0; cn < 2; ++cn) {
                    if (n < bns[cn]) continue;
                    for (int c = 0; c < 2; ++c) {
                        const long long tiles = ((M + bms[c] - 1) / bms[c]) * ((n + bns[cn] - 1) / bns[cn]);
                        const long long rounds = (tiles + 255) / 256;
                        const double fill = (double)tiles / (double)(rounds * 256);
                        const double rate = bns[cn] == 256 ? 1.0 : 0.8;
                        if (fill < 0.8 && !(concurrent && rounds == 1 && fill >= 0.4)) continue;
                        const double span = (double)rounds * bms[c] * bns[cn] / rate;
                        const double cost = concurrent ? (double)tiles * bms[c] * bns[cn] / rate : span;
                        const bool better = best_cost < 0 || (concurrent ? (cost < 0.97 * best_cost || (cost < 1.03 * best_cost && span < best_span))
                                                                         : cost < best_cost);
                        if (better) best_cost = cost, best_span = span, bm = bms[c], bn = bns[cn];
                    }
                }
                use = best_cost >= 0;
            }
            if (pp >= 2) {
                if (MCAMD_ENV_INT("MCAMD_PP_BM", 256) == 192) bm = 192;
                if (MCAMD_ENV_INT("MCAMD_PP_BN", 256) == 128) bn = 128;
            }
            if (use) {
                t.bm = bm, t.bn = bn, t.bk = 32, t.kind = 2;
                return t;
            }
        }
    }
    int best = 128, waste = round_up_int(n, 128);
    for (int bn = 64; bn >= 32; bn /= 2)
        if (round_up_int(n, bn) < waste) {
            waste = round_up_int(n, bn);
            best = bn;
        }
    t.bm = 128;
    t.bn = best;
    if (t.bn == 128 && (n % 64 == 0 || round_up_int(n, 64) == round_up_int(n, 128))) {
        const long long t128 = ((M + 127) / 128) * ((n + 127) / 128);
        if (t128 < 256 && 2 * t128 <= 512) t.bn = 64;
    }
    int want_bk = MCAMD_ENV_INT("MCAMD_BK", 64);
    t.bk = (want_bk == 64 && cin_tap % 64 == 0) ? 64 : 32;
    if (t.bm == 128 && t.bn == 128 && t.bk == 64 && ktot >= 2048) {
        const long long nt = (n + 127) / 128;
        const long long t128 = ((M + 127) / 128) * nt, t192 = ((M + 191) / 192) * nt;
        const long long cost128 = ((t128 + 511) / 512) * 128, cost192 = ((t192 + 511) / 512) * 192;
        if (cost192 <= cost128) t.bm = 192;
    }
    return t;
}

static int igemm_mtiles(long long M, int bm) { return (int)((M + bm - 1) / bm); }

ConvRoute mcamd_igemm_route(long long M, int n, int cin_tap, int ktot, bool raw_epilogue, bool concurrent) {
    const TileCfg t = pick_tile(M, n, cin_tap, ktot, raw_epilogue, concurrent);
    if (t.kind == ROUTE_SMALL3X3) return {t.kind, t.bm, t.bn, t.bk, mcamd_small3x3_rows(M)};
    int ntiles = (n + t.bn - 1) / t.bn;
    int mtiles = igemm_mtiles(M, t.bm);
    int target = t.kind == ROUTE_PP ? 256 : 2048;
    int p = target / ntiles;
    if (p < 1) p = 1;
    if (p > mtiles) p = mtiles;
// ... 61 lines not shown
```

### modelcompression_amd/csrc/kernels.h

```cpp
#pragma once
#include "common.h"

struct DgradSums {
    float* slab;
    const half_t* act;
    const float* scale;
    const float* shift;
    const float* mean;
    const float* invstd;
    const float* y;
    int act_ld, act_choff, act_pw;
    int y_ld, y_choff;
    int ch_lo, C;
    int ld;
    float slope;
};
#define MCAMD_EPI_RAW_F16_SUMS 4

struct IgemmArgs {
    const half_t* x;
    const half_t* w;
    void* y;
    const float* bias;
    float* stats;
// ... 49 lines not shown
    int dy_zero_off;
    int H, W, HW, M;
    int rows_pad;
    int ktot, cin_tap, ntaps;
    int tap_off[9];
    int n_ctiles;
    int n_otiles, n_tapgroups, nsplit;
    int pix_per_split;
};

struct WgradPlan {
    int tmo, tnc, taps, kp, rows_pad, n_otiles, n_ctiles, n_tapgroups, nsplit, pix_per_split;
    int nine;
    int stemw;
    int ns;
    size_t bytes;
};

struct WgradFinish {
    int kernel;
    int sg;
};

enum { ROUTE_IGEMM = 0, ROUTE_STEM = 1, ROUTE_PP = 2, ROUTE_SMALL3X3 = 4, ROUTE_WIN3X3 = 5, ROUTE_WRES = 6, ROUTE_SMALL3X3_SPLIT = 7 };
struct ConvRoute {
    int kernel;
    int bm, bn, bk;
    int rows;
};

ConvRoute mcamd_igemm_route(long long M, int n, int cin_tap, int ktot, bool raw_epilogue, bool concurrent);
int mcamd_igemm_pp_launch(const IgemmArgs& a, int bm, int bn, int rows, int ntiles, hipStream_t st);
int mcamd_igemm_launch(IgemmArgs& a, const ConvRoute& r, hipStream_t st);
bool mcamd_igemm_sums_ok(const ConvRoute& r);
struct SplitkPlan {
    int bm, bn, bk, chunks, mtiles, ntiles, tiles, slices;
    long long slab_elems;
};
SplitkPlan mcamd_splitk_plan(long long M, int n, int cin_tap, int ktot, int forced);
int mcamd_splitk_launch(const IgemmArgs& a, const SplitkPlan& p, float* ws, hipStream_t st);
int mcamd_sparse24_launch(IgemmArgs& a, const void* idx, hipStream_t st);
int mcamd_pack_sparse24_launch(const float* w, const float* mask, void* vals, void* idx, int cout, int cin, int ntaps,
                               int cin_tap, int kb, hipStream_t st);
int mcamd_conv_q8_launch(IgemmArgs& a, const void* wexp, int y_f8, int y2_f8, hipStream_t st, const float* border = nullptr,
                         int border_ld = 0);
int mcamd_pack_q8_launch(const float* w, const float* mask, void* wq, void* wexp, int cout, int cin, int ntaps, hipStream_t st);
int mcamd_pack_q8_slim_launch(const float* w, const float* mask, void* wq, void* wexp, int cout, int cin, int ntaps, hipStream_t st);
#define MCAMD_Q8_TILE_M 128
int mcamd_cast_q8_launch(const void* src, long long pixels, int src_ld, int src_choff, int C, void* dst, int dst_ld,
                         int dst_choff, int back, hipStream_t st);
int mcamd_fakequant_q8_launch(const float* w, const float* mask, const void* wexp, float* out, int cout, int cin, int ntaps,
                              hipStream_t st);
int mcamd_conv_q8_sparse_launch(IgemmArgs& a, const void* idx, const void* wexp, int y_f8, int y2_f8, hipStream_t st);
int mcamd_pack_q8_sparse24_launch(const float* w, const float* mask, void* wq, void* idx, void* wexp, int cout, int cin,
                                  int ntaps, hipStream_t st);

WgradPlan mcamd_wgrad_plan(long long M, int cout, int cin_tap, int ntaps);
int mcamd_wgrad_launch(WgradArgs& a, const WgradPlan& p, hipStream_t st);
bool mcamd_wgrad_stem_ok(int stem, int cout, int W, long long M);
WgradPlan mcamd_wgrad_stem_plan(long long M);
int mcamd_wgrad_stem_launch(WgradArgs& a, const WgradPlan& p, hipStream_t st);
bool mcamd_wgrad_win_ok(int ksize, int stem, int cout, int cin_tap, int W, long long M);
WgradPlan mcamd_wgrad_win_plan(long long M, int cout);
int mcamd_wgrad_win_launch(WgradArgs& a, const WgradPlan& p, hipStream_t st);
bool mcamd_wgrad_use9(int ksize, int stem, int cout, int cin_tap, int W);
WgradPlan mcamd_wgrad_plan9(long long P, int cout, int cin_tap, int W, int pitch, int B);
int mcamd_wgrad9_launch(const WgradArgs& w, const WgradPlan& p, int pitch, long long P, hipStream_t st);
WgradFinish mcamd_wgrad_finish_pick(int nsplit, int stem, int Cin, int ksize, bool has_cmap);
int mcamd_wgrad_instances(int (*out)[4], int cap);
int mcamd_wgrad_finish_launch(const float* slab, const WgradPlan& p, int ktot, int cin_tap, int stem, int Cout, int Cin,
                              int ksize, const float* mask, float inv_scale, float* dw, const int* rmap, const int* cmap,
                              hipStream_t st);
int mcamd_colsum_launch(const half_t* dy, long long rows, int ld, int choff, int C, float inv_scale, float* out,
                        hipStream_t st, void* scratch, size_t scratch_bytes);

bool mcamd_win3x3_ok(int mode, bool stats, long long M, int n, int cin_tap, int ktot, int H, int W);
int mcamd_win3x3_launch(const IgemmArgs& a, hipStream_t st);
bool mcamd_small3x3_ok(long long M, int n, int cin_tap, int ktot);
int mcamd_small3x3_rows(long long M);
int mcamd_small3x3_launch(const IgemmArgs& a, int rows, hipStream_t st);
bool mcamd_small3x3_split_ok(long long M, int n, int cin_tap, int ktot, int wrap, int mode);
int mcamd_small3x3_split_launch(const IgemmArgs& a, int rows, hipStream_t st);

bool mcamd_wres_ok(int ksize, int stem, int n, int cin_tap, int ktot, int B, int H, int W, int mode);
int mcamd_wres_rows(int n, int B, int H, int W);
int mcamd_wres_launch(IgemmArgs& a, int B, int rows, hipStream_t st);

bool mcamd_stem_direct_ok(int stem, int cout, int mode);
int mcamd_stem_rows(long long M);
int mcamd_stem_launch(const StemArgs& a, int cout, int rows, hipStream_t st);
```

### modelcompression_amd/engine.py

```python
import contextlib
import math
import os
import time

import torch

from . import ops
from . import _lib as L
from ._lib import McamdError


class _T:
    __slots__ = ("buf", "ld", "choff", "C", "H", "W", "ps", "ps0")

    def __init__(self, buf, ld, choff, C, H, W, ps=0):
        self.buf, self.ld, self.choff, self.C, self.H, self.W, self.ps = buf, ld, choff, C, H, W, ps
        self.ps0 = ps


class _Layer:
    pass


def _resolve_routes(blocks):
# ... 15 lines not shown
PLAIN_BLOCK_ERR = 2.9e-4
MIXED_BUDGET = 5.5e-4
MIXED_BUDGET_TRAIN = 7.0e-4
TRAIN_GAIN = 1.1


def _probe_side_stream(device, tries=8):
    lock = None
    try:
        import fcntl
        import tempfile
        lock = open(os.path.join(tempfile.gettempdir(), "mcamd_side_probe.lock"), "w")
        fcntl.flock(lock, fcntl.LOCK_EX)
    except Exception:
        lock = None
    try:
        main = torch.cuda.current_stream(device)
        big = torch.empty(64 << 20, dtype=torch.float32, device=device)
        tiny = torch.zeros(64, dtype=torch.float32, device=device)
        first = None
        for _ in range(tries):
            cand = torch.cuda.Stream(device)
            first = first or cand
            torch.cuda.synchronize(device)
            busy, done = torch.cuda.Event(enable_timing=True), torch.cuda.Event(enable_timing=True)
            for _ in range(80):
                big.fill_(1.0)
            busy.record(main)
            with torch.cuda.stream(cand):
                tiny.add_(1.0)
                done.record(cand)
            torch.cuda.synchronize(device)
            concurrent = done.elapsed_time(busy) > 0.0
            if concurrent:
                return cand, True
        return first, False
    finally:
        if lock is not None:
            try:
                import fcntl
                fcntl.flock(lock, fcntl.LOCK_UN)
                lock.close()
            except Exception:
                pass


class Engine:
    def __init__(self, model, B, H, W, device, grad_scale=256.0, precision="fp16", for_training=False, train_layout=False):
        if precision not in ("fp16", "fp16x3", "mixed", "fp8", "fp8-2:4", "fp8-qat"):
            raise McamdError("precision must be 'fp16', 'fp16x3', 'mixed', 'fp8', 'fp8-2:4' or 'fp8-qat' (got %r)" % (precision,))
        self.model, self.B, self.device = model, B, device
        self.precision = precision
        self.for_training = bool(for_training)
        self.train_layout = bool(train_layout)
        self.precise = precision not in ("fp16", "fp8", "fp8-2:4", "fp8-qat")
        self.q8 = precision in ("fp8", "fp8-2:4", "fp8-qat")
        self.qat = precision == "fp8-qat"
        self.fp8_layers = []
        self.q8_sparse = precision == "fp8-2:4"
        self.fp8_sparse_layers = []
        self.qbufs = {}
        self._qld = {}
        self._q8_keys = None
        self.grad_scale = float(grad_scale)
        self.serial = 0
        self._packed_sig = None
        self.events = None
        self.overlap_wgrad = os.environ.get("MCAMD_OVERLAP_WGRAD", "1") == "1"
        self.wgrad_chunk = 1
        self.use_plan = os.environ.get("MCAMD_PLAN", "1") == "1"
        self._fwd_plans, self._bwd_plan, self._plan_epoch = {}, None, 0
        self._logits = self._gout = self._flat = None
        self._pack_on_side = False
        self.sparse_layers = []
        self._sparse_mode, self._sparse_keys = None, None
        self.splitk_layers = []
        self._splitk_on, self._splitk_keys, self._splitk_ws = False, None, None
        self.fold_dead = os.environ.get("MCAMD_FOLD_DEAD", "1") == "1"
        self.f8 = precision == "mixed" and os.environ.get("MCAMD_F8", "1") == "1"
        self.bn_narrow_on = True
        self.bwd_from_act = True
        self.pool_act_on = True
        self.dgrad_bn_sums = os.environ.get("MCAMD_DGRAD_BN_SUMS", "1") == "1"
        self._dgrad_sums_cache = {}
        self._side_stream = None
        self._side_concurrent = True
        self._side_ws = None
        self.overflow = torch.zeros(1, dtype=torch.int32, device=device)
        self._build_plan(H, W)

    def _build_plan(self, H0, W0):
        model, B, dev = self.model, self.B, self.device
        blocks = model.blocks
        bops = _resolve_routes(blocks)
        n = len(bops)

        def alias(t):
            while t >= 0 and bops[t][0] == "route" and len(bops[t][1]) == 1:
                t = bops[t][1][0]
            return t

        srcs = [[alias(s) for s in o[1]] for o in bops]
        consumers = {}
        for ind, (t, _) in enumerate(bops):
            if t == "route" and len(srcs[ind]) == 1:
                continue
            for s in srcs[ind]:
                consumers.setdefault(s, []).append(ind)

        shape = {-1: (int(blocks[0]["channels"]), H0, W0)}
        for ind, (t, _) in enumerate(bops):
            if t == "convolutional":
                c, h, w = shape[srcs[ind][0]]
                assert int(blocks[ind + 1]["stride"]) == 1, "only stride-1 convolutions (YOLOv2)"
                shape[ind] = (int(blocks[ind + 1]["filters"]), h, w)
            elif t == "maxpool":
                c, h, w = shape[srcs[ind][0]]
                if int(blocks[ind + 1]["size"]) != 2 or int(blocks[ind + 1]["stride"]) != 2:
                    raise NotImplementedError("only maxpool size=2 stride=2 is on the YOLOv2 path")
                shape[ind] = (c, h // 2, w // 2)
            elif t == "reorg":
                c, h, w = shape[srcs[ind][0]]
                assert int(blocks[ind + 1]["stride"]) == 2
                shape[ind] = (4 * c, h // 2, w // 2)
            elif t == "route":
                if len(srcs[ind]) == 1:
                    shape[ind] = shape[srcs[ind][0]]
                else:
                    (c1, h, w), (c2, h2, w2) = shape[srcs[ind][0]], shape[srcs[ind][1]]
                    assert (h, w) == (h2, w2)
                    shape[ind] = (c1 + c2, h, w)

        self._bops, self._srcs, self._shape = bops, srcs, shape
        conv_inds = [i for i, (t, _) in enumerate(bops) if t == "convolutional"]
        fused = {}
        for ci in conv_inds:
            cons = consumers.get(ci, [])
            pools = [c for c in cons if bops[c][0] == "maxpool"]
            reorgs = [c for c in cons if bops[c][0] == "reorg"]
            if len(pools) == 1 and len(cons) == 1:
                fused[ci] = (L.DST_POOL, pools[0], None)
            elif len(pools) == 1 and not reorgs:
                fused[ci] = (L.DST_POOL, pools[0], ci)
            elif len(reorgs) == 1 and len(cons) == 1:
                fused[ci] = (L.DST_REORG, reorgs[0], None)
            elif not pools and not reorgs:
                fused[ci] = (L.DST_PLAIN, ci, None)
            else:
                raise NotImplementedError("unsupported consumer pattern after conv block %d" % ci)
        for ind, (t, _) in enumerate(bops):
            if t in ("maxpool", "reorg") and not any(f[1] == ind for f in fused.values()):
                raise NotImplementedError("stand-alone %s block %d (not directly after a conv)" % (t, ind))

        place = {}
        self.bufs = []

        self.shared_halo_maxw = 0
        if self.train_layout:
            self.shared_halo_maxw = 26

        def pad_for(w):
            return 1 if (w <= self.shared_halo_maxw and w >= 4) else 0

        def new_buf(Bn, h, w, ld):
            self.bufs.append(ops.alloc_padded(Bn, h, w, ld, dev, pad=pad_for(w)))
            return len(self.bufs) - 1
# ... 802 lines not shown
        for lay in self.layers:
            if lay.bn is not None:
                sig.append(lay.bn.running_mean.data_ptr())
                sig.append(lay.bn.running_var.data_ptr())
                sig.append((lay.bn.momentum, lay.bn.eps))
            if lay.conv.mask_flag:
                sig.append(lay.conv.mask.data_ptr())
        return tuple(sig)

    def forward(self, x, training):
        B = self.B
        if tuple(x.shape) != (B, self.layers[0].cin, self.layers[0].H, self.layers[0].W):
            raise McamdError("engine built for input %s, got %s" % ((B, self.layers[0].cin, self.layers[0].H, self.layers[0].W), tuple(x.shape)))
        if bool(training) != self.train_layout and self.shared_halo_maxw:
            raise McamdError("this engine was planned for %s (activation layout); build one for the other mode"
                             % ("training" if self.train_layout else "inference"))
        if training:
            for lay in self.layers:
                if lay.border is not None:
                    raise McamdError("slim models (border_bias tables) are inference-only: call model.eval()")
                if not lay.train_ok:
                    raise McamdError("conv block %d: training needs a BN channel count of 8 * (power of two), got %d"
                                     % (lay.index, lay.cout))
        if training and self.q8 and not self.qat:
            raise McamdError("precision %r is inference only (there is no fp8 training path): call model.eval() or "
                             "pick another precision for training" % (self.precision,))
        mode = None if training else getattr(self.model, "sparse", None)
        if mode is not None and (self.precise or self.q8):
            raise McamdError("sparse=%r runs in the plain-fp16 inference engine only (model.precision = 'fp16'), not %r%s"
                             % (mode, self.precision, "; 2:4 masks on the fp8 engine: model.precision = 'fp8-2:4' with "
                                "model.sparse = None" if self.q8 else ""))
        splitk = bool(getattr(self.model, "splitk", False)) and not training
        if splitk and (self.precise or self.q8):
            raise McamdError("splitk=True runs in the plain-fp16 inference engine only (model.precision = 'fp16'), not %r"
                             % (self.precision,))
        force = bool(training) or mode != self._sparse_mode or splitk != self._splitk_on
        self._sparse_mode, self._splitk_on = mode, splitk
        self.pack(force=force, training=training)
        self.serial += 1
        tin = self.layers[0].tin
        xs = x.detach().contiguous().float()
        if self.precise and not self.stem:
            l0 = self.layers[0]
            if l0.stem_split:
                ops.nchw_to_nhwc4_split(xs, l0.sh_img, l0.sh_img_lo)
            elif l0.stem_f32:
                if training:
                    ops.nchw_to_padded_split(xs, self.bufs[tin.buf], tin.ld, tin.choff, tin.ps)
                mask0 = l0.conv.mask if l0.conv.mask_flag else None
                self._timed('fwd', l0, ops.stem_conv_f32, xs, l0.conv.weight.data, mask0, l0.weff, l0.y, l0.cout,
                            l0.stats if training else None)
            else:
                ops.nchw_to_padded_split(xs, self.bufs[tin.buf], tin.ld, tin.choff, tin.ps)
        else:
            ops.nchw_to_padded(xs, self.bufs[tin.buf], tin.ld, tin.choff)
        if self._logits is None:
            self._logits = torch.empty(self.out_shape, dtype=torch.float32, device=self.device)
        main = torch.cuda.current_stream(self.device)
        side = self._get_side_stream() if self._pack_on_side else None
        if self.use_plan and self.events is None:
            key = (bool(training), main.cuda_stream, side.cuda_stream if side is not None else 0, self._plan_epoch,
                   self._ptr_sig())
            plan = self._fwd_plans.get(bool(training))
            if plan is None or plan.key != key:
                plan = ops.Plan([main] + ([side] if side is not None else []))
                with plan:
                    self._forward_body(training, main, side)
                plan.key = key
                self._fwd_plans[bool(training)] = plan
            plan.run()
        else:
            self._forward_body(training, main, side)
        last = self.layers[-1]
        out = self._logits + last.border_map if last.border_map is not None else self._logits.clone()
        if training:
            bns = [lay.bn.num_batches_tracked for lay in self.layers if lay.bn is not None]
            if bns:
                torch._foreach_add_(bns, 1)
        return out

    def _forward_body(self, training, main, side):
        B = self.B
        out = self._logits
        for lay in self.layers:
            xin = self.bufs[lay.tin.buf]
            if lay.li == 1 and side is not None:
                ops.stream_wait(main, side)
            if lay.is_last:
                bias = lay.conv.bias.data if lay.conv.bias is not None else None
                self._timed('fwd', lay, ops.conv_fwd_nchw, lay.geom_f if self.precise else lay.geom_act, xin, lay.wp, out, bias)
                continue
            bn = lay.bn
            if lay.fused_stem or (lay.fused_stem_eval and not training and lay.out_t.ld - lay.out_t.choff >= 32):
                if not training:
                    ops.bn_coeffs(None, lay.cout, lay.M, bn.weight.data, bn.bias.data, bn.running_mean, bn.running_var, False,
                                  lay.scale, lay.shift, lay.mean, lay.invstd, eps=bn.eps)
                t = lay.out_t
                self._timed('fwd', lay, ops.stem_block_fwd, B, lay.H, lay.W, xin, lay.wp, bn.weight.data, bn.bias.data,
                            bn.running_mean, bn.running_var, training, lay.scale, lay.shift, lay.mean, lay.invstd, lay.slope,
                            self.bufs[t.buf], t.ld, t.choff, lay.stem_ws if lay.fused_stem else None,
                            momentum=bn.momentum if bn.momentum is not None else 0.1, eps=bn.eps, cout=lay.cout,
                            planes=self.act_planes)
                continue
            if training and lay.stem_split:
                c = lay.sh_coef
                ops.stem_block_fwd(B, lay.H, lay.W, lay.sh_img, lay.sh_wp, bn.weight.data, bn.bias.data, None, None, True,
                                   c[0], c[1], c[2], c[3], lay.slope, None, 0, 0, lay.stem_ws,
                                   momentum=0.0, eps=bn.eps, cout=lay.cout, planes=1)
                self._timed('fwd', lay, self._stem_split_forward, lay)
                continue
            if self.precise:
                if not lay.stem_f32:
                    self._timed('fwd', lay, ops.conv_fwd_raw32, lay.geom_f, xin, lay.wp, lay.y, lay.cout, 0,
                                lay.stats if training else None)
                ops.bn_coeffs(lay.stats if training else None, lay.cout, lay.M, bn.weight.data, bn.bias.data,
                              bn.running_mean, bn.running_var, training, lay.scale, lay.shift, lay.mean, lay.invstd,
                              momentum=bn.momentum if bn.momentum is not None else 0.1, eps=bn.eps, perm=lay.perm32,
                              ones_channel=lay.ones_idx)
                t, t2 = lay.out_t, lay.out2_t
                af = getattr(lay, "act_full", None) if (training and self.pool_act_on) else None
                ops.bn_act_fwd(B, lay.H, lay.W, lay.bn_width or lay.cout, lay.y, lay.cout, 0, lay.scale, lay.shift,
                               lay.slope, lay.mode, self.bufs[t.buf], t.ld, t.choff,
                               self.bufs[t2.buf] if t2 is not None else None,
                               t2.ld if t2 is not None else 0, t2.choff if t2 is not None else 0, border=lay.border,
                               planes=self._planes_for(lay.out_id), dst_plane=t.ps, dst2_plane=t2.ps if t2 is not None else 0,
                               dst_pad=self._pad_for(t.W), dst2_pad=self._pad_for(t2.W) if t2 is not None else 0,
                               planes2=self._planes_for(lay.out2_id) if t2 is not None else 0,
                               pool_act=af, pool_act_ld=ops.round_up(lay.cout, 8) if af is not None else 0,
                               pool_act_pad=self._pad_for(lay.W) if af is not None else 0)
                continue
            if not training and (self._fused_eval(lay) or (self.q8 and lay.q8_on)):
                ops.bn_coeffs(None, lay.cout, lay.M, bn.weight.data, bn.bias.data, bn.running_mean, bn.running_var, False,
                              lay.scale, lay.shift, lay.mean, lay.invstd, eps=bn.eps)
                t, t2 = lay.out_t, lay.out2_t
                q8 = self.q8 and lay.q8_on
                y2 = None if t2 is None else (self.qbufs if q8 and lay.q8_y2 else self.bufs)[t2.buf]
                dst = dict(dst_mode=lay.mode, y2=y2, y2_ld=self._q8_tld(t2, q8 and lay.q8_y2) if t2 is not None else 0,
                           y2_choff=t2.choff if t2 is not None else 0)
                if q8:
                    x8 = self.qbufs.get(lay.tin.buf)
                    if lay.xq is not None:
                        ti, x8 = lay.tin, lay.xq
                        self._timed('cast', lay, ops.cast_q8, xin, B * (ti.H + 2) * (ti.W + 2), ti.ld, ti.choff, lay.cin,
                                    x8, lay.geom_q8.x_ld, ti.choff)
                    y, y_ld = (self.qbufs[t.buf] if lay.q8_y else self.bufs[t.buf]), self._q8_tld(t, lay.q8_y)
                    if lay.q8s_on:
                        self._timed('fwd', lay, ops.conv_fwd_q8_sparse24, lay.geom_q8, x8, lay.wqs, lay.widx8, lay.wexp, y,
                                    y_ld, t.choff, lay.scale, lay.shift, lay.slope, y_f8=lay.q8_y, y2_f8=lay.q8_y2, **dst)
                        continue
                    if lay.q8_slim:
                        self._timed('fwd', lay, ops.conv_fwd_q8_slim, lay.geom_q8, x8, lay.wq, lay.wexp, y, y_ld, t.choff,
                                    lay.scale, lay.shift, lay.slope, y_f8=lay.q8_y, y2_f8=lay.q8_y2, border=lay.border,
                                    border_ld=lay.cout, **dst)
                        continue
                    self._timed('fwd', lay, ops.conv_fwd_q8, lay.geom_q8, x8, lay.wq, lay.wexp, y, y_ld, t.choff, lay.scale,
                                lay.shift, lay.slope, y_f8=lay.q8_y, y2_f8=lay.q8_y2, **dst)
                    continue
                if lay.sp_on:
                    self._timed('fwd', lay, ops.conv_fwd_sparse24, lay.geom_act, xin, lay.wsp, lay.widx, self.bufs[t.buf], t.ld,
                                t.choff, lay.scale, lay.shift, lay.slope, **dst)
                    continue
                if lay.sk_on:
                    self._timed('fwd', lay, ops.conv_fwd_splitk, lay.geom_act, xin, lay.wp, self.bufs[t.buf], t.ld, t.choff,
                                lay.scale, lay.shift, lay.slope, slices=lay.sk_slices, workspace=self._splitk_ws, **dst)
                    continue
                self._timed('fwd', lay, ops.conv_fwd_padded, lay.geom_act, xin, lay.wp, self.bufs[t.buf], t.ld, t.choff,
                            lay.scale, lay.shift, lay.slope, **dst)
                continue
            if training and self._qat_train(lay):
                self._qat_forward(lay, xin)
                continue
            if lay.sk_on and not training:
                self._timed('fwd', lay, ops.conv_fwd_raw_splitk, lay.geom_act, xin, lay.wp, lay.y, lay.cout, 0,
                            slices=lay.sk_slices, workspace=self._splitk_ws)
            else:
                self._timed('fwd', lay, ops.conv_fwd_raw, lay.geom_act, xin, lay.wp, lay.y, lay.cout, 0, lay.stats if training else None)
            ops.bn_coeffs(lay.stats if training else None, lay.cout, lay.M, bn.weight.data, bn.bias.data,
                          bn.running_mean, bn.running_var, training, lay.scale, lay.shift, lay.mean, lay.invstd,
                          momentum=bn.momentum if bn.momentum is not None else 0.1, eps=bn.eps, perm=lay.perm32,
                          ones_channel=lay.ones_idx)
            t, t2 = lay.out_t, lay.out2_t
            ops.bn_act_fwd(B, lay.H, lay.W, lay.bn_width or lay.cout, lay.y, lay.cout, 0, lay.scale, lay.shift,
                           lay.slope, lay.mode, self.bufs[t.buf], t.ld, t.choff,
                           self.bufs[t2.buf] if t2 is not None else None,
                           t2.ld if t2 is not None else 0, t2.choff if t2 is not None else 0, border=lay.border,
                           dst_pad=self._pad_for(t.W), dst2_pad=self._pad_for(t2.W) if t2 is not None else 0)

    def _qat_forward(self, lay, xin):
        B, bn = self.B, lay.bn
        x8 = self.qbufs.get(lay.tin.buf)
        if lay.xq is not None:
            ti, x8 = lay.tin, lay.xq
            self._timed('cast', lay, ops.cast_q8, xin, ops.padded_pixels(B, ti.H, ti.W, self._pad_for(ti.W)), ti.ld, ti.choff,
                        lay.cin, x8, ti.ld, ti.choff, write_back=True)
        self._timed('fwd', lay, ops.conv_fwd_q8_raw, lay.geom_act, x8, lay.wq, lay.wexp, lay.y, lay.cout, 0, lay.stats)
        ops.bn_coeffs(lay.stats, lay.cout, lay.M, bn.weight.data, bn.bias.data, bn.running_mean, bn.running_var, True,
                      lay.scale, lay.shift, lay.mean, lay.invstd, momentum=bn.momentum if bn.momentum is not None else 0.1,
                      eps=bn.eps)
        t, t2 = lay.out_t, lay.out2_t
        ops.bn_act_fwd(B, lay.H, lay.W, lay.cout, lay.y, lay.cout, 0, lay.scale, lay.shift, lay.slope, lay.mode,
                       self.bufs[t.buf], t.ld, t.choff, self.bufs[t2.buf] if t2 is not None else None,
                       t2.ld if t2 is not None else 0, t2.choff if t2 is not None else 0,
                       dst_pad=self._pad_for(t.W), dst2_pad=self._pad_for(t2.W) if t2 is not None else 0,
                       dst_q8=self.qbufs[t.buf] if lay.q8_y else None,
                       dst2_q8=self.qbufs[t2.buf] if (t2 is not None and lay.q8_y2) else None)

    def _stem_split_forward(self, lay):
        bn, t = lay.bn, lay.out_t
        ops.stem_block_stats(self.B, lay.H, lay.W, lay.sh_img, lay.sh_wp, lay.stats, x_lo=lay.sh_img_lo, wp_lo=lay.sh_wp_lo)
        ops.bn_coeffs(lay.stats, lay.cout, lay.M, bn.weight.data, bn.bias.data, bn.running_mean, bn.running_var, True,
                      lay.scale, lay.shift, lay.mean, lay.invstd, momentum=bn.momentum if bn.momentum is not None else 0.1,
                      eps=bn.eps)
        ops.stem_block_fwd(self.B, lay.H, lay.W, lay.sh_img, lay.sh_wp, bn.weight.data, bn.bias.data, None, None, False,
                           lay.scale, lay.shift, lay.mean, lay.invstd, lay.slope, self.bufs[t.buf], t.ld, t.choff, None,
                           eps=bn.eps, cout=lay.cout, planes=self.act_planes, x_lo=lay.sh_img_lo, wp_lo=lay.sh_wp_lo)

    def _dgrad_sums(self, lay, concurrent):
        if not (self.dgrad_bn_sums and self.bwd_from_act and self.precise) or lay.gin is None:
            return None
        key = (lay.li, bool(concurrent), self._plan_epoch)
        hit = self._dgrad_sums_cache.get(key, False)
        if hit is not False:
            return hit
        res = None
        if lay.fold is None and not lay.gather and lay.in_perm is None and lay.geom_act is lay.geom:
            for prod in self.layers:
                if prod.is_last or prod.fused_stem or prod.stem_shadow or prod.bn is None or prod.out_t is None:
                    continue
                if self.consumer_of.get(prod.out_id) is not lay or prod.mode != L.DST_PLAIN or prod.slope <= 0.0:
                    continue
                if prod.out2_id is not None and prod.out2_id in self.consumer_of:
                    continue
                if (prod.keep is not None or prod.perm is not None or prod.fold is not None or prod.skip_dead or prod.fold_consumers
                        or prod.bn_width or prod.border is not None or prod.cout % 8 != 0):
                    continue
                t = prod.out_t
                ch_lo = t.choff - lay.tin.choff
                if t.buf != lay.tin.buf or t.ld != lay.tin.ld or ch_lo < 0 or ch_lo % 8 != 0 or ch_lo + prod.cout > lay.geom.cin:
                    continue
                rows = ops.dgrad_sums_rows(lay.geom_act, concurrent)
                if rows <= 0:
                    continue
                slab = torch.empty(rows, 2, prod.cout, dtype=torch.float32, device=self.device)
                y = prod.y if (prod.y is not None and prod.y.dtype == torch.float32) else None
                desc = ops.dgrad_sums(slab, self.bufs[t.buf], t.ld, t.choff, self._pad_for(t.W), prod.scale, prod.shift, prod.mean,
                                      prod.invstd, prod.slope, prod.cout, ch_lo=ch_lo, y=y, y_ld=prod.cout, y_choff=0)
                res = (desc, slab, prod)
                break
        self._dgrad_sums_cache = {k: v for k, v in self._dgrad_sums_cache.items() if k[2] == self._plan_epoch}
        self._dgrad_sums_cache[key] = res
        return res

    def bn_act_bwd_layer(self, lay, g, g_ld, g_choff, g2, g2_ld, g2_choff, dy, dgamma, dbeta, grad_scale, sums=None):
        cb = lay.bn_width or lay.cout
        act = {}
        if self.bwd_from_act and self.precise and lay.mode == L.DST_PLAIN and g2 is None:
            t = lay.out_t
            act = dict(act=self.bufs[t.buf], act_ld=t.ld, act_choff=t.choff, act_pad=self._pad_for(t.W))
        elif self.bwd_from_act and self.precise and self.train_layout and lay.mode == L.DST_POOL and lay.slope > 0.0:
            if self.pool_act_on and getattr(lay, "act_full", None) is not None:
                act = dict(act=lay.act_full, act_ld=ops.round_up(lay.cout, 8), act_choff=0, act_pad=self._pad_for(lay.W))
            if g2 is None and lay.y is not None:
                t = lay.out_t
                act.update(pool_out=self.bufs[t.buf], pool_out_ld=t.ld, pool_out_choff=t.choff,
                           pool_out_pad=self._pad_for(t.W))
        if sums is not None:
            act["sums"] = sums
        ops.bn_act_bwd(self.B, lay.H, lay.W, cb, lay.y, lay.cout, 0, lay.scale, lay.shift, lay.mean,
                       lay.invstd, lay.slope, lay.mode, g, g_ld, g_choff, dy, lay.cout_p, 0,
                       dgamma, dbeta, grad_scale, g2, g2_ld, g2_choff,
# ... 157 lines not shown
```

### modelcompression_amd/ops.py

```python
import collections
import ctypes as C
import weakref

import torch

from . import _lib as L
from ._lib import (ConvGeom, ConvEpilogue, SplitkInfo, ActDesc, ActBwdDesc, DgradSums, ChanMap, PackJob, StemBlockDesc, FoldDesc, FoldJob, check, ptr,
                   stream_ptr)

HALF = torch.float16
SLACK = 64


def round_up(v, m):
    return (v + m - 1) // m * m


def _need_cuda(*ts):
    for t in ts:
        if t is not None and not t.is_cuda:
            raise L.McamdError("modelcompression_amd compute ops need CUDA (MI355X) tensors; there is no CPU path")


def guard_elems(W, ld):
# ... 209 lines not shown
def wgrad_plan_info(g, has_cmap=False):
    out = (C.c_int32 * L.WGRAD_PLAN_INFO_N)()
    check(L.lib().mcamd_conv_wgrad_plan_info(C.byref(g), 1 if has_cmap else 0, out), "mcamd_conv_wgrad_plan_info")
    return WgradPlanInfo(*out)


def wgrad_generic_instances():
    lib = L.lib()
    n = int(lib.mcamd_wgrad_generic_instances(None, 0))
    out = (C.c_int32 * (4 * n))()
    lib.mcamd_wgrad_generic_instances(out, n)
    return [tuple(out[4 * i:4 * i + 4]) for i in range(n)]


def conv_wgrad(g, x, dy, dy_ld, dy_choff, dw, mask=None, grad_scale=1.0, dbias=None, workspace=None, rows=None, cols=None):
    if workspace is None:
        workspace = torch.empty(wgrad_workspace_bytes(g), dtype=torch.uint8, device=dw.device)
    check(L.lib().mcamd_conv_wgrad(C.byref(g), ptr(x), ptr(dy), dy_ld, dy_choff, ptr(mask), _chan_map(g, rows, cols), grad_scale, ptr(dw),
                                   ptr(dbias), ptr(workspace), workspace.numel(), stream_ptr()), "mcamd_conv_wgrad")


def _perm_ptr(perm, C_):
    if perm is None:
        return None
    if perm.dtype != torch.int32 or perm.numel() != C_ or not perm.is_contiguous() or not perm.is_cuda:
        raise L.McamdError("channel permutation must be a contiguous CUDA int32 vector of %d entries" % C_)
    return perm.data_ptr()


def bn_coeffs(stats, C_, count, gamma, beta, rmean, rvar, training, scale, shift, mean=None, invstd=None,
              momentum=0.1, eps=1e-5, perm=None, ones_channel=-1):
    rows = stats.shape[0] if stats is not None else 0
    ld = stats.shape[2] if stats is not None else 0
    check(L.lib().mcamd_bn_coeffs_ex(ptr(stats), rows, ld, C_, count, ptr(gamma), ptr(beta), ptr(rmean), ptr(rvar),
                                     momentum, eps, 1 if training else 0, ptr(scale), ptr(shift), ptr(mean), ptr(invstd),
                                     _perm_ptr(perm, C_), ones_channel, stream_ptr()), "mcamd_bn_coeffs_ex")


def _fold_desc(w, mask, rows, cols, beta, slope, n, cin_k, aug):
    _need_cuda(w, mask, rows, cols, beta)
    assert w.dtype == torch.float32 and w.is_contiguous() and w.dim() == 4 and w.shape[2] == w.shape[3]
    assert beta.dtype == torch.float32 and beta.numel() == w.shape[1]
    d = FoldDesc()
    d.w = w.data_ptr()
    d.mask = mask.data_ptr() if mask is not None else None
    for name, v, cnt in (("rows", rows, n), ("cols", cols, w.shape[1])):
        if v is not None:
            if v.dtype != torch.int32 or not v.is_contiguous() or v.numel() != cnt:
                raise L.McamdError("fold: channel map `%s` must be a contiguous CUDA int32 vector of %d entries" % (name, cnt))
            setattr(d, name, v.data_ptr())
    d.beta, d.slope = beta.data_ptr(), slope
    assert aug.dtype == torch.float32 and aug.is_contiguous() and aug.dim() == 4 and aug.shape[0] == n and aug.shape[1] > cin_k
    d.n, d.cin_t, d.cin_k, d.cin_aug, d.ksize = n, w.shape[1], cin_k, aug.shape[1], w.shape[2]
    return d


def fold_weights(w, mask, rows, cols, beta, slope, n, cin_k, waug):
    d = _fold_desc(w, mask, rows, cols, beta, slope, n, cin_k, waug)
    check(L.lib().mcamd_fold_weights(C.byref(d), ptr(waug), stream_ptr()), "mcamd_fold_weights")


def fold_table(jobs, device):
    arr = (FoldJob * len(jobs))()
    total = 0
    for a, j in zip(arr, jobs):
        a.d = _fold_desc(j["w"], j["mask"], j["rows"], j["cols"], j["beta"], j["slope"], j["n"], j["cin_k"], j["waug"])
        a.waug = j["waug"].data_ptr()
        a.first_block = total
        total += j["n"]
    host = torch.frombuffer(bytearray(bytes(arr)), dtype=torch.uint8)
    return host.to(device), len(jobs), total


def fold_many(table, njobs, total):
    check(L.lib().mcamd_fold_weights_many(ptr(table), njobs, total, stream_ptr()), "mcamd_fold_weights_many")


def unfold_wgrad(w, mask, rows, cols, beta, slope, n, cin_k, dwaug, dw, prod_dbeta, prod_dgamma, accumulate=False):
    d = _fold_desc(w, mask, rows, cols, beta, slope, n, cin_k, dwaug)
    check(L.lib().mcamd_unfold_wgrad(C.byref(d), ptr(dwaug), ptr(dw), ptr(prod_dbeta), ptr(prod_dgamma), 1 if accumulate else 0,
                                     stream_ptr()), "mcamd_unfold_wgrad")


def bn_act_fwd(B, H, W, C_, y, y_ld, y_choff, scale, shift, slope, mode, dst, dst_ld, dst_choff=0, dst2=None,
               dst2_ld=0, dst2_choff=0, border=None, planes=1, dst_plane=0, dst2_plane=0, dst_pad=0, dst2_pad=0, planes2=0,
               pool_act=None, pool_act_ld=0, pool_act_pad=0, dst_q8=None, dst2_q8=None):
    d = ActDesc()
    d.y_dtype = 1 if y.dtype == torch.float32 else 0
    d.planes, d.dst_plane, d.dst2_plane, d.planes2 = planes, dst_plane, dst2_plane, planes2
    d.dst_pad, d.dst2_pad = dst_pad, dst2_pad
    d.B, d.H, d.W, d.C = B, H, W, C_
    d.y, d.y_ld, d.y_choff = y.data_ptr(), y_ld, y_choff
    d.scale, d.shift, d.slope, d.mode = scale.data_ptr(), shift.data_ptr(), slope, mode
    d.dst, d.dst_ld, d.dst_choff = dst.data_ptr(), dst_ld, dst_choff
    d.dst2 = dst2.data_ptr() if dst2 is not None else None
    d.dst2_ld, d.dst2_choff = dst2_ld, dst2_choff
    if border is not None:
        if border.dtype != torch.float32 or tuple(border.shape) != (16, C_) or not border.is_contiguous():
            raise L.McamdError("bn_act_fwd: border table must be contiguous fp32 [16, %d]" % C_)
        d.border = border.data_ptr()
    if pool_act is not None:
        d.pool_act, d.pool_act_ld, d.pool_act_pad = pool_act.data_ptr(), pool_act_ld, pool_act_pad
    d.dst_q8 = dst_q8.data_ptr() if dst_q8 is not None else None
    d.dst2_q8 = dst2_q8.data_ptr() if dst2_q8 is not None else None
    check(L.lib().mcamd_bn_act_fwd(C.byref(d), stream_ptr()), "mcamd_bn_act_fwd")


def bn_act_bwd(B, H, W, C_, y, y_ld, y_choff, scale, shift, mean, invstd, slope, mode, g, g_ld, g_choff, dy, dy_ld,
               dy_choff, dgamma, dbeta, grad_scale=1.0, g2=None, g2_ld=0, g2_choff=0, workspace=None, dy_keep=None,
               perm=None, overflow=None, skip_dead_from=0, dy_pad=0, act=None, act_ld=0, act_choff=0, act_pad=0,
               pool_out=None, pool_out_ld=0, pool_out_choff=0, pool_out_pad=0, sums=None):
    d = ActBwdDesc()
    if sums is not None:
        assert sums.dtype == torch.float32 and sums.dim() == 3 and sums.shape[1] == 2 and sums.is_contiguous()
        d.sums, d.sums_rows, d.sums_ld = sums.data_ptr(), sums.shape[0], sums.shape[2]
    d.skip_dead_param_grads = int(skip_dead_from)
    d.dy_pad = dy_pad
    d.B, d.H, d.W, d.C = B, H, W, C_
    if act is not None:
        d.act, d.act_ld, d.act_choff, d.act_pad = act.data_ptr(), act_ld, act_choff, act_pad
    if pool_out is not None:
        d.pool_out, d.pool_out_ld, d.pool_out_choff, d.pool_out_pad = pool_out.data_ptr(), pool_out_ld, pool_out_choff, pool_out_pad
    d.y, d.y_ld, d.y_choff = (y.data_ptr() if y is not None else None), y_ld, y_choff
    d.scale, d.shift, d.mean, d.invstd = scale.data_ptr(), shift.data_ptr(), mean.data_ptr(), invstd.data_ptr()
    d.slope, d.mode = slope, mode
    d.g, d.g_ld, d.g_choff = g.data_ptr(), g_ld, g_choff
    d.g2 = g2.data_ptr() if g2 is not None else None
    d.g2_ld, d.g2_choff = g2_ld, g2_choff
    d.dy, d.dy_ld, d.dy_choff = dy.data_ptr(), dy_ld, dy_choff
    d.dgamma = dgamma.data_ptr() if dgamma is not None else None
    d.dbeta = dbeta.data_ptr() if dbeta is not None else None
    d.grad_scale = grad_scale
    d.dy_keep = dy_keep.data_ptr() if dy_keep is not None else None
    d.chan_perm = _perm_ptr(perm, C_)
    d.y_dtype = 1 if (y is not None and y.dtype == torch.float32) else 0
    d.overflow = overflow.data_ptr() if overflow is not None else None
    need = int(L.lib().mcamd_bn_act_bwd_workspace_bytes(C.byref(d)))
    if workspace is None:
        workspace = torch.empty(need, dtype=torch.uint8, device=g.device)
    check(L.lib().mcamd_bn_act_bwd(C.byref(d), ptr(workspace), workspace.numel(), stream_ptr()), "mcamd_bn_act_bwd")


def bn_act_bwd_workspace_bytes(C_):
    d = ActBwdDesc()
    d.C = C_
    return int(L.lib().mcamd_bn_act_bwd_workspace_bytes(C.byref(d)))


def stem_block_workspace_bytes():
    return int(L.lib().mcamd_stem_block_workspace_bytes())


def _stem_desc(B, H, W, x, wp, gamma, beta, scale, shift, mean, invstd, slope):
    _need_cuda(x, wp, scale, shift)
    d = StemBlockDesc()
    d.B, d.H, d.W = B, H, W
    d.x, d.wp = x.data_ptr(), wp.data_ptr()
    d.gamma = gamma.data_ptr() if gamma is not None else None
    d.beta = beta.data_ptr() if beta is not None else None
    d.scale, d.shift = scale.data_ptr(), shift.data_ptr()
    d.save_mean = mean.data_ptr() if mean is not None else None
    d.save_invstd = invstd.data_ptr() if invstd is not None else None
    d.slope = slope
    return d


def stem_block_fwd(B, H, W, x, wp, gamma, beta, rmean, rvar, training, scale, shift, mean, invstd, slope, dst, dst_ld,
                   dst_choff, workspace, momentum=0.1, eps=1e-5, cout=32, planes=1, x_lo=None, wp_lo=None):
    d = _stem_desc(B, H, W, x, wp, gamma, beta, scale, shift, mean, invstd, slope)
    d.running_mean = rmean.data_ptr() if rmean is not None else None
    d.running_var = rvar.data_ptr() if rvar is not None else None
    d.momentum, d.eps, d.training = momentum, eps, 1 if training else 0
    d.cout, d.planes = cout, planes
    d.dst, d.dst_ld, d.dst_choff = (dst.data_ptr() if dst is not None else None), dst_ld, dst_choff
    d.x_lo = x_lo.data_ptr() if x_lo is not None else None
    d.wp_lo = wp_lo.data_ptr() if wp_lo is not None else None
    check(L.lib().mcamd_stem_block_fwd(C.byref(d), ptr(workspace), workspace.numel() if workspace is not None else 0,
                                       stream_ptr()), "mcamd_stem_block_fwd")


def stem_block_stats_rows(B, H, W):
    d = StemBlockDesc()
    d.B, d.H, d.W = B, H, W
    return int(L.lib().mcamd_stem_block_stats_rows(C.byref(d)))


def stem_block_stats(B, H, W, x, wp, stats, x_lo=None, wp_lo=None):
    _need_cuda(x, wp, stats)
# ... 548 lines not shown
```

Measured before the change: 5575.

## Fuse BN+leaky activation producer into following 1x1 convolution forward

Adds a kernel that reads the producer's raw fp32 conv output, applies BN scale/shift and leaky ReLU, splits the result into hi/lo fp16 planes in registers, and feeds them directly into the consumer 1x1 igemm MFMA loop. It still writes the hi plane for the backward pass, but skips the separate bn_act_fwd launch and the consumer's reload of the activation planes. The engine detects eligible producer/consumer pairs, caches the decision per plan epoch, and skips the consumer's normal forward. In exchange the fused path only covers narrow shapes (cin a multiple of 64 up to 256, cout up to 128), the lo plane is never written to memory, and correctness depends on nothing else reading those planes.

```diff
diff --git a/include/mcamd.h b/include/mcamd.h
--- a/include/mcamd.h
+++ b/include/mcamd.h
@@ -208,6 +208,11 @@
     void* dst2_q8;
 } mcamd_act_desc;
 int mcamd_bn_act_fwd(const mcamd_act_desc* d, void* stream);
+
+int32_t mcamd_bn_act_conv1x1_ok(const mcamd_act_desc* d, const mcamd_conv_geom* g);
+int32_t mcamd_bn_act_conv1x1_stats_rows(const mcamd_act_desc* d, const mcamd_conv_geom* g);
+int mcamd_bn_act_conv1x1_fwd(const mcamd_act_desc* d, const mcamd_conv_geom* g, const void* wp_fwd,
+                             const mcamd_conv_epilogue* epi, void* stream);
 
 typedef struct mcamd_act_bwd_desc {
     int32_t B, H, W, C;
diff --git a/modelcompression_amd/_lib.py b/modelcompression_amd/_lib.py
--- a/modelcompression_amd/_lib.py
+++ b/modelcompression_amd/_lib.py
@@ -198,6 +198,9 @@
     "mcamd_fold_weights_many": (C.c_int, [_P, _I32, _I64, _P]),
     "mcamd_unfold_wgrad": (C.c_int, [C.POINTER(FoldDesc), _P, _P, _P, _P, _I32, _P]),
     "mcamd_bn_act_fwd": (C.c_int, [C.POINTER(ActDesc), _P]),
+    "mcamd_bn_act_conv1x1_ok": (_I32, [C.POINTER(ActDesc), C.POINTER(ConvGeom)]),
+    "mcamd_bn_act_conv1x1_stats_rows": (_I32, [C.POINTER(ActDesc), C.POINTER(ConvGeom)]),
+    "mcamd_bn_act_conv1x1_fwd": (C.c_int, [C.POINTER(ActDesc), C.POINTER(ConvGeom), _P, C.POINTER(ConvEpilogue), _P]),
     "mcamd_bn_act_bwd_workspace_bytes": (_SZ, [C.POINTER(ActBwdDesc)]),
     "mcamd_bn_act_bwd": (C.c_int, [C.POINTER(ActBwdDesc), _P, _SZ, _P]),
     "mcamd_stem_block_workspace_bytes": (_SZ, []),
diff --git a/modelcompression_amd/build.py b/modelcompression_amd/build.py
--- a/modelcompression_amd/build.py
+++ b/modelcompression_amd/build.py
@@ -27,6 +27,7 @@
     "conv_wgrad.hip": [],
     "conv_wgrad_stem.hip": [],
     "bn_act.hip": [],
+    "bn_conv1x1.hip": [],
     "fold.hip": [],
     "plan.hip": [],
     "region_loss.hip": [],
diff --git a/modelcompression_amd/csrc/api.hip b/modelcompression_amd/csrc/api.hip
--- a/modelcompression_amd/csrc/api.hip
+++ b/modelcompression_amd/csrc/api.hip
@@ -1,6 +1,8 @@
 #include <stdarg.h>
 #include <stdlib.h>
 #include <string.h>
+
+#include <string>
 
 #include "kernels.h"
 
@@ -541,6 +543,63 @@
     return launch_route(a, r, g, (hipStream_t)stream);
 }
 
+static const char* bn_conv1x1_refusal(const mcamd_act_desc* d, const mcamd_conv_geom* g, ConvRoute* r) {
+    if (!d || !g) return "null descriptor";
+    if (check_geom(g, "bn_act_conv1x1")) return mcamd_last_error();
+    if (g->ksize != 1 || g->stem) return "the consumer is not a 1x1 convolution";
+    if (g->x_f8 != 0) return "fp8 correction operands (x_f8)";
+    if (g->pad != 0 || d->dst_pad != 0) return "shared-halo destination";
+    const int P = g->x_wrap / 2;
+    if (g->x_wrap <= 0 || g->cin != 3 * P) return "the consumer does not multiply split operands on two planes (x_wrap)";
+    if (P % 64 != 0) return "input channels must be a multiple of 64";
+    if (!mcamd_bn_conv1x1_shape_ok(P, g->cout)) return "no kernel instance: cout <= 128 in steps of 8, cin <= 128 (cout <= 64) or 256";
+    if (d->mode != MCAMD_DST_PLAIN || d->dst2 || d->pool_act || d->dst_q8 || d->dst2_q8) return "the producer is not a PLAIN block with one destination";
+    if (d->border) return "border table";
+    if (d->B != g->B || d->H != g->H || d->W != g->W) return "producer and consumer differ in B x H x W";
+    if (d->C != P || d->planes != 2 || d->dst_plane != P || d->dst_ld != g->x_ld || d->dst_choff != g->x_choff)
+        return "the producer's hi | lo planes are not the consumer's input slice";
+    if (d->y_dtype != 1 || d->y_ld % 4 != 0 || d->y_choff % 4 != 0 || d->y_choff + P > d->y_ld) return "the raw output must be an fp32 slice in steps of 4 channels";
+    *r = conv_route(g, DIR_FWD, MCAMD_EPI_RAW_F32, MCAMD_DST_PLAIN, true);
+    if (r->kernel != ROUTE_IGEMM || r->bm != 128 || r->bn < 64) return "the consumer's own forward does not take 128-pixel igemm tiles in wave rows of 64";
+    return nullptr;
+}
+
+extern "C" int32_t mcamd_bn_act_conv1x1_ok(const mcamd_act_desc* d, const mcamd_conv_geom* g) {
+    ConvRoute r;
+    return bn_conv1x1_refusal(d, g, &r) ? 0 : 1;
+}
+
+extern "C" int32_t mcamd_bn_act_conv1x1_stats_rows(const mcamd_act_desc* d, const mcamd_conv_geom* g) {
+    ConvRoute r;
+    return bn_conv1x1_refusal(d, g, &r) ? 0 : r.rows;
+}
+
+extern "C" int mcamd_bn_act_conv1x1_fwd(const mcamd_act_desc* d, const mcamd_conv_geom* g, const void* wp_fwd,
+                                        const mcamd_conv_epilogue* epi, void* stream) {
+    if (mcamd_recording()) {
+        MCAMD_REQUIRE(d && g && epi, "bn_act_conv1x1_fwd: null descriptor / geometry / epilogue");
+        const mcamd_act_desc d_ = *d;
+        const mcamd_conv_geom g_ = *g;
+        const mcamd_conv_epilogue e_ = *epi;
+        return mcamd_rec_push(stream, [=](void* s) { return mcamd_bn_act_conv1x1_fwd(&d_, &g_, wp_fwd, &e_, s); });
+    }
+    ConvRoute r;
+    const char* why = bn_conv1x1_refusal(d, g, &r);
+    if (why) {
+        const std::string w(why);
+        mcamd_set_error("bn_act_conv1x1_fwd: %s (mcamd_bn_act_conv1x1_ok)", w.c_str());
+        return MCAMD_EINVAL;
+    }
+    MCAMD_REQUIRE(d->y && d->scale && d->shift && d->dst && wp_fwd && epi, "bn_act_conv1x1_fwd: null input / epilogue");
+    MCAMD_REQUIRE(epi->mode == MCAMD_EPI_RAW_F32, "bn_act_conv1x1_fwd: epilogue mode 3 (MCAMD_EPI_RAW_F32) only");
+    IgemmArgs a;
+    fill_operand(a, g, d->dst, wp_fwd, g->x_ld, g->x_choff, g->cout, cin_tap_of(g), 0);
+    a.wrap = g->x_wrap;
+    if (fill_epilogue(a, epi, g->cout, "bn_act_conv1x1_fwd", r.rows)) return MCAMD_EINVAL;
+    a.scale = d->scale, a.shift = d->shift, a.slope = d->slope;
+    return mcamd_bn_conv1x1_launch(a, (const float*)d->y, d->y_ld, d->y_choff, g->x_wrap / 2, r.rows, (hipStream_t)stream);
+}
+
 extern "C" int32_t mcamd_conv_fwd_sparse24_ok(const mcamd_conv_geom* g) {
     if (!g || g->stem || g->x_wrap != 0 || g->x_f8 != 0 || (g->ksize != 1 && g->ksize != 3)) return 0;
     if (g->B <= 0 || g->H <= 0 || g->W <= 0 || g->cin <= 0 || g->cout <= 0) return 0;
diff --git a/modelcompression_amd/csrc/bn_act.hip b/modelcompression_amd/csrc/bn_act.hip
--- a/modelcompression_amd/csrc/bn_act.hip
+++ b/modelcompression_amd/csrc/bn_act.hip
@@ -95,9 +95,6 @@
 #pragma unroll
     for (int i = 0; i < 8; ++i) v[i] = (float)h[i];
 }
-__device__ __forceinline__ half_t sat_half(float v) {
-    return (half_t)fminf(fmaxf(v, -65504.f), 65504.f);
-}
 __device__ __forceinline__ void store8(half_t* p, const float* v) {
     h8_t h;
 #pragma unroll
@@ -119,9 +116,8 @@
 }
 template <int PL>
 __device__ __forceinline__ void store_act(half_t* p, int plane, const float* v, int ci = 0) {
-    h8_t hi;
-#pragma unroll
-    for (int i = 0; i < 8; ++i) hi[i] = sat_half(v[i]);
+    h8_t hi, lo;
+    split_hi_lo(v, hi, lo);
     *(h8_t*)p = hi;
     if (PL == 4) {
         float ql[8], q8[8];
@@ -143,9 +139,6 @@
         *(i32x2_t*)b = i32x2_t{wl[0], wl[1]};
         *(i32x2_t*)(b + plane) = i32x2_t{w8[0], w8[1]};
     } else if (PL >= 2) {
-        h8_t lo;
-#pragma unroll
-        for (int i = 0; i < 8; ++i) lo[i] = (half_t)(v[i] - (float)hi[i]);
         *(h8_t*)(p + plane) = lo;
         if (PL == 3) *(h8_t*)(p + 2 * plane) = hi;
     }
@@ -210,10 +203,7 @@
                 for (int i = 0; i < 8; ++i) v[i] += bb[i];
             }
 #pragma unroll
-            for (int i = 0; i < 8; ++i) {
-                float z = v[i] * sc[i] + sh[i];
-                v[i] = z > 0.f ? z : z * a.slope;
-            }
+            for (int i = 0; i < 8; ++i) v[i] = bn_leaky(v[i], sc[i], sh[i], a.slope);
             if (Q8) store_act_q8(a.dst, a.dst_q8, pad_off(b, h, w, a.H, a.W, a.dst_ld, a.dst_pw) + a.dst_choff + c8, v);
             else store_act<PL>(a.dst + pad_off(b, h, w, a.H, a.W, a.dst_ld, a.dst_pw) + a.dst_choff + c8, a.dst_plane, v, a.dst_choff + c8);
         } else {
@@ -233,10 +223,7 @@
                     for (int i = 0; i < 8; ++i) act[k][i] += bb[i];
                 }
 #pragma unroll
-                for (int i = 0; i < 8; ++i) {
-                    float z = act[k][i] * sc[i] + sh[i];
-                    act[k][i] = z > 0.f ? z : z * a.slope;
-                }
+                for (int i = 0; i < 8; ++i) act[k][i] = bn_leaky(act[k][i], sc[i], sh[i], a.slope);
                 if (Q8) {
                     if (a.dst2) store_act_q8(a.dst2, a.dst2_q8, pad_off(b, h, w, a.H, a.W, a.dst2_ld, a.dst2_pw) + a.dst2_choff + c8, act[k]);
                 } else if (a.dst2) store_act2<PL>(a.dst2_pl, a.dst2 + pad_off(b, h, w, a.H, a.W, a.dst2_ld, a.dst2_pw) + a.dst2_choff + c8, a.dst2_plane, act[k], a.dst2_choff + c8);
diff --git a/modelcompression_amd/csrc/bn_conv1x1.hip b/modelcompression_amd/csrc/bn_conv1x1.hip
--- /dev/null
+++ b/modelcompression_amd/csrc/bn_conv1x1.hip
@@ -0,0 +1,177 @@
+#include "kernels.h"
+#include "conv_epi.h"
+
+template <int BN, int CB>
+__global__ __launch_bounds__(4 * BN, BN >= 128 ? 2 : 3)
+void bn_conv1x1_kernel(IgemmArgs a, const float* __restrict__ py, int py_ld, int py_choff) {
+    constexpr int BM = 128, WM = 64, WN = 32, BK = 64, CPR = BK / 8;
+    constexpr int WAVES_N = BN / WN;
+    constexpr int NT = (BM / WM) * WAVES_N * 64;
+    constexpr int RSTEP = NT / 8;
+    constexpr int RG = BM / RSTEP;
+    constexpr int KP = CB * RG;
+    constexpr int A_SLOTS = BM * CPR, B_SLOTS = BN * CPR;
+    constexpr int B_IT = B_SLOTS / NT;
+    constexpr int STAGE_BYTES = (A_SLOTS + B_SLOTS) * 16;
+    constexpr int NCH = 3 * CB;
+    constexpr int TM = WM / 32, TN = WN / 32;
+    static_assert(KP <= 8, "hi and lo of a thread's pieces stay in 64 registers");
+    static_assert(B_SLOTS % NT == 0 && RSTEP * RG == BM, "whole waves per DMA instruction, whole pieces per thread");
+
+    extern __shared__ __attribute__((aligned(16))) char smem[];
+
+    const int tid = threadIdx.x;
+    const int lane = tid & 63;
+    const int wave = __builtin_amdgcn_readfirstlane(tid >> 6);
+    const int wm = wave / WAVES_N, wn = wave % WAVES_N;
+    int nt, pslot;
+    if (!xcd_tile(1, a.num_pslots, nt, pslot)) return;
+    const int j8 = tid & 7, rsub = tid >> 3;
+
+    long long bbase[B_IT];
+#pragma unroll
+    for (int it = 0; it < B_IT; ++it) {
+        int slot = it * NT + tid;
+        int row = slot / CPR, phys = slot % CPR;
+        bbase[it] = (long long)row * a.ktot + (phys ^ swz<CPR>(row)) * 8;
+    }
+
+    float s1[TN], s2[TN];
+#pragma unroll
+    for (int j = 0; j < TN; ++j) s1[j] = s2[j] = 0.f;
+
+    for (int mt = pslot; mt < a.num_mtiles; mt += a.num_pslots) {
+        f32x4_t raw[KP][2];
+        half_t* hdst[RG];
+        bool real[RG];
+#pragma unroll
+        for (int rg = 0; rg < RG; ++rg) {
+            const int m = mt * BM + rg * RSTEP + rsub;
+            const int mc = m < a.M ? m : a.M - 1;
+            real[rg] = m < a.M;
+            hdst[rg] = (half_t*)a.x + tile_x_base(a, false, m) + a.tap_off[0] + j8 * 8;
+            const float* src = py + (long long)mc * py_ld + py_choff + j8 * 8;
+#pragma unroll
+            for (int cb = 0; cb < CB; ++cb) {
+                raw[cb * RG + rg][0] = *(const f32x4_t*)(src + cb * 64);
+                raw[cb * RG + rg][1] = *(const f32x4_t*)(src + cb * 64 + 4);
+            }
+        }
+        h8_t hi[KP], lo[KP];
+#pragma unroll
+        for (int cb = 0; cb < CB; ++cb) {
+            const float *scp = pin_here(a.scale) + cb * 64 + j8 * 8, *shp = pin_here(a.shift) + cb * 64 + j8 * 8;
+            const f32x4_t sc0 = *(const f32x4_t*)scp, sc1 = *(const f32x4_t*)(scp + 4);
+            const f32x4_t sh0 = *(const f32x4_t*)shp, sh1 = *(const f32x4_t*)(shp + 4);
+#pragma unroll
+            for (int rg = 0; rg < RG; ++rg) {
+                const int k = cb * RG + rg;
+                float v[8];
+#pragma unroll
+                for (int i = 0; i < 4; ++i) {
+                    v[i] = bn_leaky(raw[k][0][i], sc0[i], sh0[i], a.slope);
+                    v[4 + i] = bn_leaky(raw[k][1][i], sc1[i], sh1[i], a.slope);
+                }
+                split_hi_lo(v, hi[k], lo[k]);
+                if (real[rg]) *(h8_t*)(hdst[rg] + cb * 64) = hi[k];
+            }
+        }
+
+        f32x16_t acc[TM][TN];
+#pragma unroll
+        for (int i = 0; i < TM; ++i)
+#pragma unroll
+            for (int j = 0; j < TN; ++j)
+#pragma unroll
+                for (int r = 0; r < 16; ++r) acc[i][j][r] = 0.f;
+
+        auto stage = [&](int q, int buf) {
+            char* sa = smem + buf * STAGE_BYTES;
+            char* sb = sa + A_SLOTS * 16;
+#pragma unroll
+            for (int it = 0; it < B_IT; ++it)
+                glds16(a.w + bbase[it] + (long long)q * BK, sb + (it * NT + wave * 64) * 16);
+            const int part = q / CB, cb = q - part * CB;
+#pragma unroll
+            for (int rg = 0; rg < RG; ++rg) {
+                const int row = rg * RSTEP + rsub;
+                *(h8_t*)(sa + (row * CPR + (j8 ^ swz<CPR>(row))) * 16) = part == 1 ? lo[cb * RG + rg] : hi[cb * RG + rg];
+            }
+        };
+
+        __syncthreads();
+        stage(0, 0);
+#pragma unroll
+        for (int q = 0; q < NCH; ++q) {
+            __syncthreads();
+            if (q + 1 < NCH) stage(q + 1, (q + 1) & 1);
+            const char* sa = smem + (q & 1) * STAGE_BYTES;
+            const char* sb = sa + A_SLOTS * 16;
+            constexpr int KS = BK / 16;
+            h8_t af[2][TM], bf[2][TN];
+            auto load_frags = [&](int s, int set) {
+                const int chunk = 2 * s + (lane >> 5);
+#pragma unroll
+                for (int i = 0; i < TM; ++i) {
+                    int row = wm * WM + i * 32 + (lane & 31);
+                    af[set][i] = *(const h8_t*)(sa + (row * CPR + (chunk ^ swz<CPR>(row))) * 16);
+                }
+#pragma unroll
+                for (int j = 0; j < TN; ++j) {
+                    int row = wn * WN + j * 32 + (lane & 31);
+                    bf[set][j] = *(const h8_t*)(sb + (row * CPR + (chunk ^ swz<CPR>(row))) * 16);
+                }
+            };
+            load_frags(0, 0);
+#pragma unroll
+            for (int s = 0; s < KS; ++s) {
+                if (s + 1 < KS) load_frags(s + 1, (s + 1) & 1);
+                __builtin_amdgcn_sched_barrier(0);
+#pragma unroll
+                for (int i = 0; i < TM; ++i)
+#pragma unroll
+                    for (int j = 0; j < TN; ++j)
+                        acc[i][j] = __builtin_amdgcn_mfma_f32_32x32x16_f16(af[s & 1][i], bf[s & 1][j], acc[i][j], 0, 0, 0);
+                __builtin_amdgcn_sched_barrier(0);
+            }
+        }
+        store_raw32_tile<BM, BN, WM, WN>(a, acc, mt, nt, wm, wn, lane, s1, s2);
+    }
+    if (a.stats) store_stats_slab<BM, BN, WM, WN, NT>(a, smem, s1, s2, pslot, nt, wm, wn, lane, tid);
+}
+
+bool mcamd_bn_conv1x1_shape_ok(int P, int cout) {
+    if (P <= 0 || P % 64 != 0 || cout <= 0 || cout > 128 || cout % 8 != 0) return false;
+    return P <= 2 * (cout <= 64 ? 64 : 128);
+}
+
+template <int BN, int CB>
+static void launch_bc(const IgemmArgs& a, const float* py, int py_ld, int py_choff, hipStream_t st) {
+    constexpr int NT = 4 * BN;
+    const size_t lds = 2 * (size_t)(128 + BN) * 8 * 16;
+    if (lds > 64 * 1024) MCAMD_LDS_OPT_IN((bn_conv1x1_kernel<BN, CB>), lds);
+    hipLaunchKernelGGL((bn_conv1x1_kernel<BN, CB>), dim3(round_up_int(a.num_pslots, 8) + 8), dim3(NT), lds, st, a, py, py_ld, py_choff);
+}
+
+int mcamd_bn_conv1x1_launch(IgemmArgs& a, const float* py, int py_ld, int py_choff, int P, int rows, hipStream_t st) {
+    if (!mcamd_bn_conv1x1_shape_ok(P, a.N) || a.ktot != 3 * P) {
+        mcamd_set_error("bn_act_conv1x1: no kernel instance for %d -> %d channels", P, a.N);
+        return MCAMD_EINVAL;
+    }
+    a.num_mtiles = (a.M + 127) / 128;
+    a.num_pslots = rows;
+    a.num_ntiles = 1;
+    a.xcd_order = 1;
+    const int cb = P / 64;
+    if (a.N <= 64) {
+        if (cb == 1) launch_bc<64, 1>(a, py, py_ld, py_choff, st);
+        else launch_bc<64, 2>(a, py, py_ld, py_choff, st);
+    } else {
+        if (cb == 1) launch_bc<128, 1>(a, py, py_ld, py_choff, st);
+        else if (cb == 2) launch_bc<128, 2>(a, py, py_ld, py_choff, st);
+        else if (cb == 3) launch_bc<128, 3>(a, py, py_ld, py_choff, st);
+        else launch_bc<128, 4>(a, py, py_ld, py_choff, st);
+    }
+    MCAMD_LAUNCH_CHECK("bn_act_conv1x1");
+    return MCAMD_OK;
+}
diff --git a/modelcompression_amd/csrc/conv_epi.h b/modelcompression_amd/csrc/conv_epi.h
--- a/modelcompression_amd/csrc/conv_epi.h
+++ b/modelcompression_amd/csrc/conv_epi.h
@@ -153,6 +153,72 @@
         const int n0 = nt * COLS + ch * 8;
         if (m < a.M && n0 < a.N) *(h8_t*)(y + (long long)m * a.y_ld + a.y_choff + n0) = *(const h8_t*)(ct + row * COLS + ch * 8);
     }
+}
+
+template <int BM, int BN, int WM, int WN>
+__device__ __forceinline__ void store_raw32_tile(const IgemmArgs& __restrict__ a, const f32x16_t (&acc)[WM / 32][WN / 32], int mt, int nt,
+                                                 int wm, int wn, int lane, float (&s1)[WN / 32], float (&s2)[WN / 32]) {
+    constexpr int TM = WM / 32, TN = WN / 32;
+    float* y = (float*)a.y;
+    const int mlim = a.M - mt * BM;
+#pragma unroll
+    for (int j = 0; j < TN; ++j) {
+        const int n = nt * BN + wn * WN + j * 32 + (lane & 31);
+#pragma unroll
+        for (int i = 0; i < TM; ++i)
+#pragma unroll
+            for (int r = 0; r < 16; ++r) {
+                const int row = wm * WM + i * 32 + mfma32_row(r, lane);
+                const float v = acc[i][j][r];
+                if (row < mlim) {
+                    if (n < a.N) y[(long long)(mt * BM + row) * a.y_ld + a.y_choff + n] = v;
+                    s1[j] += v;
+                    s2[j] += v * v;
+                }
+            }
+    }
+}
+
+template <int BM, int BN, int WM, int WN, int NT>
+__device__ __forceinline__ void store_stats_slab(const IgemmArgs& __restrict__ a, char* smem, float (&s1)[WN / 32], float (&s2)[WN / 32],
+                                                 int pslot, int nt, int wm, int wn, int lane, int tid) {
+    constexpr int TN = WN / 32;
+#pragma unroll
+    for (int j = 0; j < TN; ++j) {
+        s1[j] += __shfl_xor(s1[j], 32);
+        s2[j] += __shfl_xor(s2[j], 32);
+    }
+    __syncthreads();
+    float* red = (float*)smem;
+    if (lane < 32) {
+#pragma unroll
+        for (int j = 0; j < TN; ++j) {
+            red[(wm * 2 + 0) * BN + wn * WN + j * 32 + lane] = s1[j];
+            red[(wm * 2 + 1) * BN + wn * WN + j * 32 + lane] = s2[j];
+        }
+    }
+    __syncthreads();
+    for (int t = tid; t < 2 * BN; t += NT) {
+        int which = t / BN, col = t - which * BN;
+        float v = 0.f;
+#pragma unroll
+        for (int k = 0; k < BM / WM; ++k) v += red[(k * 2 + which) * BN + col];
+        a.stats[((long long)pslot * 2 + which) * a.stats_ld + nt * BN + col] = v;
+    }
+}
+
+__device__ __forceinline__ float bn_leaky(float y, float sc, float sh, float slope) {
+    const float z = y * sc + sh;
+    return z > 0.f ? z : z * slope;
+}
+__device__ __forceinline__ half_t sat_half(float v) {
+    return (half_t)fminf(fmaxf(v, -65504.f), 65504.f);
+}
+__device__ __forceinline__ void split_hi_lo(const float* v, h8_t& hi, h8_t& lo) {
+#pragma unroll
+    for (int i = 0; i < 8; ++i) hi[i] = sat_half(v[i]);
+#pragma unroll
+    for (int i = 0; i < 8; ++i) lo[i] = (half_t)(v[i] - (float)hi[i]);
 }
 
 template <class T>
diff --git a/modelcompression_amd/csrc/conv_igemm.hip b/modelcompression_amd/csrc/conv_igemm.hip
--- a/modelcompression_amd/csrc/conv_igemm.hip
+++ b/modelcompression_amd/csrc/conv_igemm.hip
@@ -173,24 +173,7 @@
                     }
                 }
         } else if constexpr (EPI == MCAMD_EPI_RAW_F32) {
-            float* y = (float*)a.y;
-            const int mlim = a.M - mt * BM;
-#pragma unroll
-            for (int j = 0; j < TN; ++j) {
-                const int n = nt * BN + wn * WN + j * 32 + (lane & 31);
-#pragma unroll
-                for (int i = 0; i < TM; ++i)
-#pragma unroll
-                    for (int r = 0; r < 16; ++r) {
-                        const int row = wm * WM + i * 32 + mfma32_row(r, lane);
-                        const float v = acc[i][j][r];
-                        if (row < mlim) {
-                            if (n < a.N) y[(long long)(mt * BM + row) * a.y_ld + a.y_choff + n] = v;
-                            s1[j] += v;
-                            s2[j] += v * v;
-                        }
-                    }
-            }
+            store_raw32_tile<BM, BN, WM, WN>(a, acc, mt, nt, wm, wn, lane, s1, s2);
         } else {
             h8_t aq[SUMS ? sums_early(BM, BN, NT) : 1];
             if constexpr (SUMS) sums_prefetch<BM, BN, NT>(a, mt, nt, tid, aq);
@@ -237,30 +220,8 @@
 
     if (sat && a.overflow) atomicOr(a.overflow, 1);
     if constexpr (SUMS) store_tile_sums_slab<BN, NT>(a, pslot, nt, tid, tot);
-    if ((EPI == MCAMD_EPI_RAW_F16 || EPI == MCAMD_EPI_RAW_F32) && a.stats) {
-#pragma unroll
-        for (int j = 0; j < TN; ++j) {
-            s1[j] += __shfl_xor(s1[j], 32);
-            s2[j] += __shfl_xor(s2[j], 32);
-        }
-        __syncthreads();
-        float* red = (float*)smem;
-        if (lane < 32) {
-#pragma unroll
-            for (int j = 0; j < TN; ++j) {
-                red[(wm * 2 + 0) * BN + wn * WN + j * 32 + lane] = s1[j];
-                red[(wm * 2 + 1) * BN + wn * WN + j * 32 + lane] = s2[j];
-            }
-        }
-        __syncthreads();
-        for (int t = tid; t < 2 * BN; t += NT) {
-            int which = t / BN, col = t - which * BN;
-            float v = 0.f;
-#pragma unroll
-            for (int k = 0; k < BM / WM; ++k) v += red[(k * 2 + which) * BN + col];
-            a.stats[((long long)pslot * 2 + which) * a.stats_ld + nt * BN + col] = v;
-        }
-    }
+    if ((EPI == MCAMD_EPI_RAW_F16 || EPI == MCAMD_EPI_RAW_F32) && a.stats)
+        store_stats_slab<BM, BN, WM, WN, NT>(a, smem, s1, s2, pslot, nt, wm, wn, lane, tid);
 }
 
 struct TileCfg {
diff --git a/modelcompression_amd/csrc/kernels.h b/modelcompression_amd/csrc/kernels.h
--- a/modelcompression_amd/csrc/kernels.h
+++ b/modelcompression_amd/csrc/kernels.h
@@ -155,6 +155,9 @@
 bool mcamd_small3x3_split_ok(long long M, int n, int cin_tap, int ktot, int wrap, int mode);
 int mcamd_small3x3_split_launch(const IgemmArgs& a, int rows, hipStream_t st);
 
+bool mcamd_bn_conv1x1_shape_ok(int P, int cout);
+int mcamd_bn_conv1x1_launch(IgemmArgs& a, const float* py, int py_ld, int py_choff, int P, int rows, hipStream_t st);
+
 bool mcamd_wres_ok(int ksize, int stem, int n, int cin_tap, int ktot, int B, int H, int W, int mode);
 int mcamd_wres_rows(int n, int B, int H, int W);
 int mcamd_wres_launch(IgemmArgs& a, int B, int rows, hipStream_t st);
diff --git a/modelcompression_amd/engine.py b/modelcompression_amd/engine.py
--- a/modelcompression_amd/engine.py
+++ b/modelcompression_amd/engine.py
@@ -121,6 +121,9 @@
         self.bwd_from_act = True
         self.pool_act_on = True
         self.dgrad_bn_sums = os.environ.get("MCAMD_DGRAD_BN_SUMS", "1") == "1"
+        self.fuse_bn_1x1 = os.environ.get("MCAMD_FUSE_BN_1X1", "1") == "1"
+        self.fused_1x1_launches = 0
+        self._fused_1x1_cache = {}
         self._dgrad_sums_cache = {}
         self._side_stream = None
         self._side_concurrent = True
@@ -1089,6 +1092,7 @@
     def _forward_body(self, training, main, side):
         B = self.B
         out = self._logits
+        fused_done = set()
         for lay in self.layers:
             xin = self.bufs[lay.tin.buf]
             if lay.li == 1 and side is not None:
@@ -1117,7 +1121,7 @@
                 self._timed('fwd', lay, self._stem_split_forward, lay)
                 continue
             if self.precise:
-                if not lay.stem_f32:
+                if not lay.stem_f32 and lay.li not in fused_done:
                     self._timed('fwd', lay, ops.conv_fwd_raw32, lay.geom_f, xin, lay.wp, lay.y, lay.cout, 0,
                                 lay.stats if training else None)
                 ops.bn_coeffs(lay.stats if training else None, lay.cout, lay.M, bn.weight.data, bn.bias.data,
@@ -1125,6 +1129,13 @@
                               momentum=bn.momentum if bn.momentum is not None else 0.1, eps=bn.eps, perm=lay.perm32,
                               ones_channel=lay.ones_idx)
                 t, t2 = lay.out_t, lay.out2_t
+                cons = self._fused_1x1(lay)
+                if cons is not None:
+                    self._timed('fwd', cons, ops.bn_act_conv1x1_fwd, *self._fused_1x1_act(lay), cons.geom_f, cons.wp, cons.y,
+                                cons.cout, 0, cons.stats if training else None)
+                    fused_done.add(cons.li)
+                    self.fused_1x1_launches += 1
+                    continue
                 af = getattr(lay, "act_full", None) if (training and self.pool_act_on) else None
                 ops.bn_act_fwd(B, lay.H, lay.W, lay.bn_width or lay.cout, lay.y, lay.cout, 0, lay.scale, lay.shift,
                                lay.slope, lay.mode, self.bufs[t.buf], t.ld, t.choff,
@@ -1193,6 +1204,40 @@
                            t2.ld if t2 is not None else 0, t2.choff if t2 is not None else 0, border=lay.border,
                            dst_pad=self._pad_for(t.W), dst2_pad=self._pad_for(t2.W) if t2 is not None else 0)
 
+    def _fused_1x1_act(self, lay):
+        t = lay.out_t
+        return ((self.B, lay.H, lay.W, lay.cout, lay.y, lay.cout, 0, lay.scale, lay.shift, lay.slope, lay.mode,
+                 self.bufs[t.buf], t.ld, t.choff),
+                dict(planes=self._planes_for(lay.out_id), dst_plane=t.ps, dst_pad=self._pad_for(t.W)))
+
+    def _fused_1x1(self, lay):
+        if not (self.fuse_bn_1x1 and self.precise):
+            return None
+        key = (lay.li, self._plan_epoch)
+        hit = self._fused_1x1_cache.get(key, False)
+        if hit is not False:
+            return hit
+        res = None
+        cons = self.consumer_of.get(lay.out_id)
+        t = lay.out_t
+        if (cons is not None and t is not None and lay.mode == L.DST_PLAIN and lay.out2_id is None and lay.out2_t is None
+                and not lay.stem and not lay.fused_stem and not lay.stem_split and not lay.stem_f32
+                and lay.keep is None and lay.perm is None and lay.fold is None and not lay.fold_consumers and not lay.bn_width
+                and not lay.skip_dead and lay.ones_idx < 0 and lay.border is None
+                and lay.y is not None and lay.y.dtype == torch.float32
+                and cons.bn is not None and not cons.is_last and cons.k == 1 and cons.level == 3 and not cons.f8
+                and cons.fold is None and not cons.gather and cons.in_perm is None and cons.geom_act is cons.geom
+                and cons.src == lay.out_id
+                and cons.tin.buf == t.buf and cons.tin.ld == t.ld and cons.tin.choff == t.choff and cons.cin == lay.cout
+                and cons.y is not None and cons.y.dtype == torch.float32):
+            args, kw = self._fused_1x1_act(lay)
+            d = ops.act_geom(self.B, lay.H, lay.W, lay.cout, lay.cout, 0, lay.slope, lay.mode, t.ld, t.choff, **kw)
+            if ops.bn_act_conv1x1_ok(d, cons.geom_f):
+                res = cons
+        self._fused_1x1_cache = {k: v for k, v in self._fused_1x1_cache.items() if k[1] == self._plan_epoch}
+        self._fused_1x1_cache[key] = res
+        return res
+
     def _qat_forward(self, lay, xin):
         B, bn = self.B, lay.bn
         x8 = self.qbufs.get(lay.tin.buf)
diff --git a/modelcompression_amd/ops.py b/modelcompression_amd/ops.py
--- a/modelcompression_amd/ops.py
+++ b/modelcompression_amd/ops.py
@@ -315,9 +315,9 @@
                                      stream_ptr()), "mcamd_unfold_wgrad")
 
 
-def bn_act_fwd(B, H, W, C_, y, y_ld, y_choff, scale, shift, slope, mode, dst, dst_ld, dst_choff=0, dst2=None,
-               dst2_ld=0, dst2_choff=0, border=None, planes=1, dst_plane=0, dst2_plane=0, dst_pad=0, dst2_pad=0, planes2=0,
-               pool_act=None, pool_act_ld=0, pool_act_pad=0, dst_q8=None, dst2_q8=None):
+def _act_desc(B, H, W, C_, y, y_ld, y_choff, scale, shift, slope, mode, dst, dst_ld, dst_choff=0, dst2=None,
+              dst2_ld=0, dst2_choff=0, border=None, planes=1, dst_plane=0, dst2_plane=0, dst_pad=0, dst2_pad=0, planes2=0,
+              pool_act=None, pool_act_ld=0, pool_act_pad=0, dst_q8=None, dst2_q8=None):
     d = ActDesc()
     d.y_dtype = 1 if y.dtype == torch.float32 else 0
     d.planes, d.dst_plane, d.dst2_plane, d.planes2 = planes, dst_plane, dst2_plane, planes2
@@ -336,7 +336,43 @@
         d.pool_act, d.pool_act_ld, d.pool_act_pad = pool_act.data_ptr(), pool_act_ld, pool_act_pad
     d.dst_q8 = dst_q8.data_ptr() if dst_q8 is not None else None
     d.dst2_q8 = dst2_q8.data_ptr() if dst2_q8 is not None else None
+    return d
+
+
+def bn_act_fwd(B, H, W, C_, y, y_ld, y_choff, scale, shift, slope, mode, dst, dst_ld, dst_choff=0, dst2=None,
+               dst2_ld=0, dst2_choff=0, border=None, planes=1, dst_plane=0, dst2_plane=0, dst_pad=0, dst2_pad=0, planes2=0,
+               pool_act=None, pool_act_ld=0, pool_act_pad=0, dst_q8=None, dst2_q8=None):
+    d = _act_desc(**locals())
     check(L.lib().mcamd_bn_act_fwd(C.byref(d), stream_ptr()), "mcamd_bn_act_fwd")
+
+
+class _NoPtr:
+    dtype = torch.float32
+
+    @staticmethod
+    def data_ptr():
+        return None
+
+
+def act_geom(B, H, W, C_, y_ld, y_choff, slope, mode, dst_ld, dst_choff=0, **kw):
+    return _act_desc(B, H, W, C_, _NoPtr, y_ld, y_choff, _NoPtr, _NoPtr, slope, mode, _NoPtr, dst_ld, dst_choff, **kw)
+
+
+def bn_act_conv1x1_ok(d, g):
+    return bool(L.lib().mcamd_bn_act_conv1x1_ok(C.byref(d), C.byref(g)))
+
+
+def bn_act_conv1x1_stats_rows(d, g):
+    return int(L.lib().mcamd_bn_act_conv1x1_stats_rows(C.byref(d), C.byref(g)))
+
+
+def bn_act_conv1x1_fwd(act_args, act_kw, g, wp, y, y_ld, y_choff=0, stats=None):
+    d = _act_desc(*act_args, **act_kw)
+    e = _epi(L.EPI_RAW_F32, y, y_ld, y_choff, stats=stats,
+             stats_rows_=stats.shape[0] if stats is not None else 0,
+             stats_ld=stats.shape[2] if stats is not None else 0)
+    check(L.lib().mcamd_bn_act_conv1x1_fwd(C.byref(d), C.byref(g), ptr(wp), C.byref(e), stream_ptr()),
+          "mcamd_bn_act_conv1x1_fwd")
 
 
 def bn_act_bwd(B, H, W, C_, y, y_ld, y_choff, scale, shift, mean, invstd, slope, mode, g, g_ld, g_choff, dy, dy_ld,
```

After: 5631 (median of 6 runs). +1.0%, better.
